# Ced3-han/PepFlowww

Hardware: AMD Instinct MI355X
Metric: residues x denoise-steps / s (higher is better)
Workload: dtype f32 (fp32 storage and accumulation; matrix products as 3 x f16 split MFMA, ~22-bit operands); 1 GPU; cfg4/GPU: B=64 x 128-residue synthetic pockets (112 ctx + 16 gen) per GPU; per_gpu_batch=64, residues=128, global_batch=64, parallelism=batch-shard x1, hipgraph=True, precision=fp32

## Files before the change

### pepflowww_amd/csrc/common.h

```cpp
#pragma once
#include <hip/hip_runtime.h>

static inline int pf_cu_count() {
    static int cache[64] = {0};
    int dev = 0, c = 256;
    if (hipGetDevice(&dev) != hipSuccess) return 256;
    if (dev >= 0 && dev < 64 && cache[dev] > 0) return cache[dev];
    if (hipDeviceGetAttribute(&c, hipDeviceAttributeMultiprocessorCount, dev) != hipSuccess || c <= 0) c = 256;
    if (dev >= 0 && dev < 64) cache[dev] = c;
    return c;
}
#include <stdint.h>

#define PF_WAVE 64

typedef float f32x4 __attribute__((ext_vector_type(4)));

__device__ __forceinline__ f32x4 mfma16(float a, float b, f32x4 c) {
    return __builtin_amdgcn_mfma_f32_16x16x4f32(a, b, c, 0, 0, 0);
}

__device__ __forceinline__ void lds_barrier() {
    asm volatile("s_waitcnt lgkmcnt(0)" ::: "memory");
    __builtin_amdgcn_s_barrier();
    asm volatile("" ::: "memory");
}

template <int CTRL, int BANK = 0xF>
__device__ __forceinline__ float dpp_mov(float old, float v) {
    return __int_as_float(__builtin_amdgcn_update_dpp(__float_as_int(old), __float_as_int(v), CTRL, 0xF, BANK, false));
}
__device__ __forceinline__ float lane_xor1(float v) { return dpp_mov<0xB1>(v, v); }
__device__ __forceinline__ float lane_xor2(float v) { return dpp_mov<0x4E>(v, v); }
__device__ __forceinline__ float lane_xor4(float v) {
    float t = dpp_mov<0x104, 0x5>(v, v);
    return dpp_mov<0x114, 0xA>(t, v);
}
__device__ __forceinline__ float lane_xor8(float v) { return dpp_mov<0x128>(v, v); }
template <int OFF> __device__ __forceinline__ float lane_xor(float v) {
    if constexpr (OFF == 1) return lane_xor1(v);
    else if constexpr (OFF == 2) return lane_xor2(v);
    else if constexpr (OFF == 4) return lane_xor4(v);
    else return lane_xor8(v);
}
__device__ __forceinline__ float sum_xor16(float v) {
    auto r = __builtin_amdgcn_permlane16_swap(__float_as_uint(v), __float_as_uint(v), false, false);
    return __uint_as_float(r[0]) + __uint_as_float(r[1]);
}
__device__ __forceinline__ float sum_xor32(float v) {
    auto r = __builtin_amdgcn_permlane32_swap(__float_as_uint(v), __float_as_uint(v), false, false);
    return __uint_as_float(r[0]) + __uint_as_float(r[1]);
}
__device__ __forceinline__ float max_xor16(float v) {
    auto r = __builtin_amdgcn_permlane16_swap(__float_as_uint(v), __float_as_uint(v), false, false);
    return fmaxf(__uint_as_float(r[0]), __uint_as_float(r[1]));
}
__device__ __forceinline__ float max_xor32(float v) {
    auto r = __builtin_amdgcn_permlane32_swap(__float_as_uint(v), __float_as_uint(v), false, false);
    return fmaxf(__uint_as_float(r[0]), __uint_as_float(r[1]));
}
__device__ __forceinline__ bool pf_rows_all_masked(const int* __restrict__ key_end, int L, int m0, int n, int M) {
    if (!key_end) return false;
    const int mend = m0 + n < M ? m0 + n : M;
    int m = m0;
    while (m < mend) {
        const int b = m / L, i = m - b * L;
        if (i < key_end[b]) return false;
        m = (b + 1) * L;
    }
    return true;
}
__device__ __forceinline__ float row16_sum(float v) {
    v += lane_xor8(v); v += lane_xor4(v); v += lane_xor2(v); v += lane_xor1(v);
    return v;
}
__device__ __forceinline__ float row16_max(float v) {
    v = fmaxf(v, lane_xor8(v)); v = fmaxf(v, lane_xor4(v)); v = fmaxf(v, lane_xor2(v)); v = fmaxf(v, lane_xor1(v));
    return v;
}
__device__ __forceinline__ float wave_sum(float v) { return sum_xor32(sum_xor16(row16_sum(v))); }
__device__ __forceinline__ float wave_max(float v) { return max_xor32(max_xor16(row16_max(v))); }

__device__ __forceinline__ float keep_if(bool ok, float v) { return __uint_as_float(__float_as_uint(v) & (ok ? 0xffffffffu : 0u)); }
__device__ __forceinline__ float4 keep_if(bool ok, const float4& v) {
    const unsigned m = ok ? 0xffffffffu : 0u;
    return make_float4(__uint_as_float(__float_as_uint(v.x) & m), __uint_as_float(__float_as_uint(v.y) & m),
                       __uint_as_float(__float_as_uint(v.z) & m), __uint_as_float(__float_as_uint(v.w) & m));
}

template <int MT, int NT>
__device__ __forceinline__ void mfma_slice(const float4 (&a)[MT], const float4 (&b)[NT], f32x4 (&acc)[MT][NT]) {
#pragma unroll
    for (int mt = 0; mt < MT; ++mt)
#pragma unroll
        for (int nt = 0; nt < NT; ++nt) {
            acc[mt][nt] = mfma16(a[mt].x, b[nt].x, acc[mt][nt]);
            acc[mt][nt] = mfma16(a[mt].y, b[nt].y, acc[mt][nt]);
            acc[mt][nt] = mfma16(a[mt].z, b[nt].z, acc[mt][nt]);
            acc[mt][nt] = mfma16(a[mt].w, b[nt].w, acc[mt][nt]);
        }
}

template <int NT, int PF_DEPTH = 4>
struct BStream {
    const float* wrow[NT];
    bool wok[NT];
    float4 ring[PF_DEPTH][NT];
    int nslices;

    __device__ __forceinline__ void init(const float* __restrict__ W, int ldw, int n0, int n_valid, int K) {
        const int lane = threadIdx.x & 63;
        const int r = lane & 15, g = lane >> 4;
        nslices = K >> 4;
#pragma unroll
        for (int nt = 0; nt < NT; ++nt) {
            const int n = n0 + 16 * nt + r;
            wok[nt] = n < n_valid;
            wrow[nt] = W + (size_t)(wok[nt] ? n : 0) * ldw + 4 * g;
        }
    }
    __device__ __forceinline__ void load(int slot_static, int slice, float4 (&dst)[NT]) {
        (void)slot_static;
#pragma unroll
        for (int nt = 0; nt < NT; ++nt)
            dst[nt] = *reinterpret_cast<const float4*>(wrow[nt] + 16 * slice);
    }
    __device__ __forceinline__ void prefetch() {
#pragma unroll
        for (int d = 0; d < PF_DEPTH; ++d)
            if (d < nslices) load(d, d, ring[d]);
    }
};

template <int MT, int NT, int PF_DEPTH>
__device__ __forceinline__ void gemm_ldsA_stream(const float* __restrict__ A_lds, int lda, BStream<NT, PF_DEPTH>& bs,
                                                 f32x4 (&acc)[MT][NT], int slice0, int count) {
    const int lane = threadIdx.x & 63;
    const float* arow = A_lds + (lane & 15) * lda + 4 * (lane >> 4);
    const int ns = bs.nslices;
    for (int base = 0; base < count; base += PF_DEPTH) {
#pragma unroll
        for (int u = 0; u < PF_DEPTH; ++u) {
            if (base + u < count) {
                const int sl = slice0 + base + u;
                float4 a[MT];
#pragma unroll
                for (int mt = 0; mt < MT; ++mt)
                    a[mt] = *reinterpret_cast<const float4*>(arow + mt * 16 * lda + 16 * (base + u));
                mfma_slice<MT, NT>(a, bs.ring[u], acc);
                if (sl + PF_DEPTH < ns) bs.load(u, sl + PF_DEPTH, bs.ring[u]);
            }
        }
    }
}

template <int MT, int NT>
__device__ __forceinline__ void gemm_ldsA_glbB(const float* __restrict__ A_lds, int lda,
                                               const float* __restrict__ W, int ldw, int n0, int n_valid,
                                               int K, f32x4 (&acc)[MT][NT]) {
    BStream<NT> bs;
    bs.init(W, ldw, n0, n_valid, K);
    bs.prefetch();
    gemm_ldsA_stream<MT, NT, 4>(A_lds, lda, bs, acc, 0, bs.nslices);
}

typedef _Float16 half8 __attribute__((ext_vector_type(8)));
typedef _Float16 half4 __attribute__((ext_vector_type(4)));
__device__ __forceinline__ float exp_softmax(float x) { return __builtin_amdgcn_exp2f(x * 1.4426950408889634f); }
constexpr float PF_LO_SCALE = 2048.f, PF_LO_INV = 1.f / 2048.f;

__device__ __forceinline__ f32x4 mfma_h(half8 a, half8 b, f32x4 c) {
    return __builtin_amdgcn_mfma_f32_16x16x32_f16(a, b, c, 0, 0, 0);
}
constexpr float PF_F16_MAX = 65504.f;
#ifndef PF_SPLIT_SATURATE
#define PF_SPLIT_SATURATE 1
#endif
__device__ __forceinline__ void split4(const float (&v)[4], half4& hi, half4& lo) {
#pragma unroll
    for (int e = 0; e < 4; ++e) {
#if PF_SPLIT_SATURATE
        const float vc = fminf(fmaxf(v[e], -PF_F16_MAX), PF_F16_MAX) + v[e] * 0.f;
#else
        const float vc = v[e];
#endif
        const _Float16 h = (_Float16)vc;
        hi[e] = h;
        lo[e] = (_Float16)__builtin_fmaf((float)h, -PF_LO_SCALE, vc * PF_LO_SCALE);
    }
}
__device__ __forceinline__ float join(f32x4 m, f32x4 c, int e) { return m[e] + c[e] * PF_LO_INV; }

template <int WT, int D, bool SP = false>
struct WSplit {
    const _Float16* wh[WT];
    const _Float16* wl[WT];
    half8 rh[D][WT], rl[D][WT];
    int nsteps;
    __device__ __forceinline__ void init(const void* planes, int Npad, int K, int n0) {
        const int lane = threadIdx.x & 63;
        const _Float16* hi = reinterpret_cast<const _Float16*>(planes);
        const _Float16* lo = hi + (size_t)Npad * K;
        nsteps = K >> 5;
#pragma unroll
        for (int wt = 0; wt < WT; ++wt) {
            const size_t off = ((size_t)((n0 >> 4) + wt) * nsteps * 64 + lane) * 8;
            wh[wt] = hi + off;
            wl[wt] = lo + off;
        }
    }
    __device__ __forceinline__ void load(int step, half8 (&dh)[WT], half8 (&dl)[WT]) {
#pragma unroll
        for (int wt = 0; wt < WT; ++wt) {
            dh[wt] = *reinterpret_cast<const half8*>(wh[wt] + (size_t)step * 512);
            if constexpr (!SP) dl[wt] = *reinterpret_cast<const half8*>(wl[wt] + (size_t)step * 512);
        }
    }
    __device__ __forceinline__ void prefetch() {
#pragma unroll
        for (int d = 0; d < D; ++d)
            if (d < nsteps) load(d, rh[d], rl[d]);
    }
};

template <int WT, int D, bool SP>
__device__ __forceinline__ void gemm_split16(WSplit<WT, D, SP>& ws, const _Float16* Xh, const _Float16* Xl, int ldx,
                                             f32x4 (&am)[WT], f32x4 (&ac)[WT], int step0, int count) {
    const int lane = threadIdx.x & 63;
    const int off = (lane & 15) * ldx + 8 * (lane >> 4);
    for (int base = 0; base < count; base += D) {
#pragma unroll
        for (int u = 0; u < D; ++u) {
            if (base + u < count) {
                const int st = step0 + base + u;
                const half8 xh = *reinterpret_cast<const half8*>(Xh + off + 32 * (base + u));
                half8 xl;
                if constexpr (!SP) xl = *reinterpret_cast<const half8*>(Xl + off + 32 * (base + u));
#pragma unroll
                for (int wt = 0; wt < WT; ++wt) {
                    am[wt] = mfma_h(ws.rh[u][wt], xh, am[wt]);
                    if constexpr (!SP) {
                        ac[wt] = mfma_h(ws.rh[u][wt], xl, ac[wt]);
                        ac[wt] = mfma_h(ws.rl[u][wt], xh, ac[wt]);
                    }
                }
                if (st + D < ws.nsteps) ws.load(st + D, ws.rh[u], ws.rl[u]);
            }
        }
    }
}
template <int WT, int D, bool SP, int RT>
__device__ __forceinline__ void gemm_split16r(WSplit<WT, D, SP>& ws, const _Float16* Xh, const _Float16* Xl, int ldx,
                                              f32x4 (&am)[RT][WT], f32x4 (&ac)[RT][WT], int step0, int count) {
    const int lane = threadIdx.x & 63;
    const int off = (lane & 15) * ldx + 8 * (lane >> 4);
    for (int base = 0; base < count; base += D) {
#pragma unroll
        for (int u = 0; u < D; ++u) {
            if (base + u < count) {
                const int st = step0 + base + u;
#pragma unroll
                for (int rt = 0; rt < RT; ++rt) {
                    const half8 xh = *reinterpret_cast<const half8*>(Xh + rt * 16 * ldx + off + 32 * (base + u));
                    half8 xl;
                    if constexpr (!SP) xl = *reinterpret_cast<const half8*>(Xl + rt * 16 * ldx + off + 32 * (base + u));
#pragma unroll
                    for (int wt = 0; wt < WT; ++wt) {
                        am[rt][wt] = mfma_h(ws.rh[u][wt], xh, am[rt][wt]);
                        if constexpr (!SP) {
                            ac[rt][wt] = mfma_h(ws.rh[u][wt], xl, ac[rt][wt]);
                            ac[rt][wt] = mfma_h(ws.rl[u][wt], xh, ac[rt][wt]);
                        }
                    }
                }
                if (st + D < ws.nsteps) ws.load(st + D, ws.rh[u], ws.rl[u]);
            }
        }
    }
}
template <int WT> __device__ __forceinline__ void acc_zero1(f32x4 (&a)[WT], f32x4 (&b)[WT]) {
#pragma unroll
    for (int wt = 0; wt < WT; ++wt) { a[wt] = (f32x4){0.f, 0.f, 0.f, 0.f}; b[wt] = (f32x4){0.f, 0.f, 0.f, 0.f}; }
}

template <int WT>
struct WPre {
    half8 h[WT], l[WT];
    __device__ __forceinline__ void load(const void* planes, int N, int Kw, int n0) {
        const int lane = threadIdx.x & 63;
        const int wsteps = Kw >> 5;
        const _Float16* wh = reinterpret_cast<const _Float16*>(planes) + ((size_t)(n0 >> 4) * wsteps * 64 + lane) * 8;
        const _Float16* wl = wh + (size_t)N * Kw;
        const size_t tstride = (size_t)wsteps * 512;
#pragma unroll
        for (int wt = 0; wt < WT; ++wt) {
            h[wt] = *reinterpret_cast<const half8*>(wh + wt * tstride);
            l[wt] = *reinterpret_cast<const half8*>(wl + wt * tstride);
        }
    }
};

template <int WT, int PT, bool SP = false>
__device__ __forceinline__ void gemm_split_lowreg(const void* planes, int N, int Kw, int n0, int K,
                                                  const _Float16* Xh, const _Float16* Xl, int ldx,
                                                  f32x4 (&am)[WT][PT], f32x4 (&ac)[WT][PT]) {
    static_assert(PT % 2 == 0, "row tiles are fed in pairs");
    const int lane = threadIdx.x & 63, r = lane & 15, g = lane >> 4;
    const int wsteps = Kw >> 5, nst = K >> 5;
    const _Float16* wh = reinterpret_cast<const _Float16*>(planes) + ((size_t)(n0 >> 4) * wsteps * 64 + lane) * 8;
    const _Float16* wl = wh + (size_t)N * Kw;
    const size_t tstride = (size_t)wsteps * 512;
    const _Float16* xh = Xh + r * ldx + 8 * g;
    const _Float16* xl = Xl + r * ldx + 8 * g;
    for (int st = 0; st < nst; ++st) {
        half8 bh[WT], bl[WT];
#pragma unroll
        for (int wt = 0; wt < WT; ++wt) {
            bh[wt] = *reinterpret_cast<const half8*>(wh + wt * tstride + (size_t)st * 512);
            if constexpr (!SP) bl[wt] = *reinterpret_cast<const half8*>(wl + wt * tstride + (size_t)st * 512);
        }
#pragma unroll
        for (int p0 = 0; p0 < PT; p0 += 2) {
            half8 ah[2], al[2];
#pragma unroll
            for (int q = 0; q < 2; ++q) {
                ah[q] = *reinterpret_cast<const half8*>(xh + (p0 + q) * 16 * ldx + 32 * st);
                if constexpr (!SP) al[q] = *reinterpret_cast<const half8*>(xl + (p0 + q) * 16 * ldx + 32 * st);
            }
#pragma unroll
            for (int wt = 0; wt < WT; ++wt)
#pragma unroll
                for (int q = 0; q < 2; ++q) am[wt][p0 + q] = mfma_h(bh[wt], ah[q], am[wt][p0 + q]);
            if constexpr (!SP) {
#pragma unroll
                for (int wt = 0; wt < WT; ++wt)
#pragma unroll
                    for (int q = 0; q < 2; ++q) ac[wt][p0 + q] = mfma_h(bh[wt], al[q], ac[wt][p0 + q]);
#pragma unroll
                for (int wt = 0; wt < WT; ++wt)
#pragma unroll
                    for (int q = 0; q < 2; ++q) ac[wt][p0 + q] = mfma_h(bl[wt], ah[q], ac[wt][p0 + q]);
            }
        }
    }
}

template <int WT, int PT, bool SWZ = false, bool SP = false, bool SWAP = false>
__device__ __forceinline__ void gemm_split(const void* planes, int N, int Kw, int n0, int K,
                                           const _Float16* Xh, const _Float16* Xl, int ldx,
                                           f32x4 (&am)[WT][PT], f32x4 (&ac)[WT][PT], const WPre<WT>* pre = nullptr) {
    const int lane = threadIdx.x & 63, r = lane & 15, g = lane >> 4;
    const int wsteps = Kw >> 5;
    const _Float16* wh = reinterpret_cast<const _Float16*>(planes) + ((size_t)(n0 >> 4) * wsteps * 64 + lane) * 8;
    const _Float16* wl = wh + (size_t)N * Kw;
    const size_t tstride = (size_t)wsteps * 512;
    const int gs = SWZ ? (g ^ ((r >> 2) & 1)) : g;
    const _Float16* xh = Xh + r * ldx + 8 * gs;
    const _Float16* xl = Xl + r * ldx + 8 * gs;
    half8 bh[WT], bl[WT], nh[WT], nl[WT];
#pragma unroll
    for (int wt = 0; wt < WT; ++wt) {
        if (pre) { bh[wt] = pre->h[wt]; bl[wt] = pre->l[wt]; }
        else {
            bh[wt] = *reinterpret_cast<const half8*>(wh + wt * tstride);
            if constexpr (!SP) bl[wt] = *reinterpret_cast<const half8*>(wl + wt * tstride);
        }
    }
    const int nst = K >> 5;
    for (int st = 0; st < nst; ++st) {
        if (st + 1 < nst) {
#pragma unroll
            for (int wt = 0; wt < WT; ++wt) {
                nh[wt] = *reinterpret_cast<const half8*>(wh + wt * tstride + (size_t)(st + 1) * 512);
                if constexpr (!SP) nl[wt] = *reinterpret_cast<const half8*>(wl + wt * tstride + (size_t)(st + 1) * 512);
            }
        }
        half8 ah[PT], al[PT];
#pragma unroll
        for (int pt = 0; pt < PT; ++pt) {
            ah[pt] = *reinterpret_cast<const half8*>(xh + pt * 16 * ldx + 32 * st);
            if constexpr (!SP) al[pt] = *reinterpret_cast<const half8*>(xl + pt * 16 * ldx + 32 * st);
        }
#pragma unroll
        for (int wt = 0; wt < WT; ++wt)
#pragma unroll
            for (int pt = 0; pt < PT; ++pt) am[wt][pt] = SWAP ? mfma_h(ah[pt], bh[wt], am[wt][pt]) : mfma_h(bh[wt], ah[pt], am[wt][pt]);
        if constexpr (!SP) {
#pragma unroll
            for (int wt = 0; wt < WT; ++wt)
#pragma unroll
                for (int pt = 0; pt < PT; ++pt) ac[wt][pt] = SWAP ? mfma_h(al[pt], bh[wt], ac[wt][pt]) : mfma_h(bh[wt], al[pt], ac[wt][pt]);
#pragma unroll
            for (int wt = 0; wt < WT; ++wt)
#pragma unroll
                for (int pt = 0; pt < PT; ++pt) ac[wt][pt] = SWAP ? mfma_h(ah[pt], bl[wt], ac[wt][pt]) : mfma_h(bl[wt], ah[pt], ac[wt][pt]);
        }
#pragma unroll
        for (int wt = 0; wt < WT; ++wt) { bh[wt] = nh[wt]; if constexpr (!SP) bl[wt] = nl[wt]; }
    }
}

__device__ __forceinline__ int swz_col(int n0, int r, int g) {
    return n0 + 8 * ((g >> 1) ^ ((r >> 2) & 1)) + 4 * (g & 1);
}

template <int MT, int NT>
__device__ __forceinline__ void acc_zero(f32x4 (&acc)[MT][NT]) {
#pragma unroll
    for (int mt = 0; mt < MT; ++mt)
#pragma unroll
        for (int nt = 0; nt < NT; ++nt) acc[mt][nt] = (f32x4){0.f, 0.f, 0.f, 0.f};
}

__device__ __forceinline__ int xcd_remap(int bid, int nblk) {
    const int q = nblk >> 3, rem = nblk & 7, x = bid & 7, k = bid >> 3;
    return (x < rem ? x * (q + 1) : rem * (q + 1) + (x - rem) * q) + k;
}

#define PF_CHECK_LAUNCH() do { hipError_t e_ = hipGetLastError(); if (e_ != hipSuccess) return (int)e_; } while (0)

struct PfOncePerDevice {
    bool done[32] = {};
    bool first() {
        int d = 0;
        (void)hipGetDevice(&d);
        d &= 31;
        if (done[d]) return false;
        done[d] = true;
        return true;
    }
};
```

### pepflowww_amd/csrc/node_track.hip

```cpp
#include "common.h"
#include "rigid_dev.h"
#include "../../include/pepflow_hip.h"

#ifdef PF_PROFILE
__device__ long long g_prof[64];
#ifndef PF_PROF_LAST
#define PF_PROF_LAST 1
#endif
#define PROF(i) do { if (LAST == (PF_PROF_LAST != 0) && blockIdx.x == 0 && threadIdx.x == 0) g_prof[i] = clock64(); } while (0)
extern "C" int pf_debug_prof(long long* out, int n) {
    return (int)hipMemcpyFromSymbol(out, HIP_SYMBOL(g_prof), sizeof(long long) * n, 0, hipMemcpyDeviceToHost);
}
#else
#define PROF(i)
#endif

namespace {

constexpr int TR = 16;
constexpr int LDX = 132;
constexpr int LDP = 136;
constexpr int NTHR = 512;
#ifndef PF_NT_MINW
#define PF_NT_MINW 2
#endif

struct Planes { _Float16* h; _Float16* l; };

struct LnParams { float g[8], b[8]; };
__device__ __forceinline__ void ln_load(LnParams& p, const float* __restrict__ g, const float* __restrict__ b) {
    const int sub = threadIdx.x & 15;
    const float4 g0 = *reinterpret_cast<const float4*>(g + 8 * sub), g1 = *reinterpret_cast<const float4*>(g + 8 * sub + 4);
    const float4 b0 = *reinterpret_cast<const float4*>(b + 8 * sub), b1 = *reinterpret_cast<const float4*>(b + 8 * sub + 4);
    p.g[0] = g0.x; p.g[1] = g0.y; p.g[2] = g0.z; p.g[3] = g0.w; p.g[4] = g1.x; p.g[5] = g1.y; p.g[6] = g1.z; p.g[7] = g1.w;
    p.b[0] = b0.x; p.b[1] = b0.y; p.b[2] = b0.z; p.b[3] = b0.w; p.b[4] = b1.x; p.b[5] = b1.y; p.b[6] = b1.z; p.b[7] = b1.w;
}
template <int ROWS = 16>
__device__ __forceinline__ void ln_tile(float* T, const LnParams& p, float mk, Planes out, int m0, int M, float* gout) {
    const int tid = threadIdx.x;
    if (tid < 16 * ROWS) {
        const int row = tid >> 4, sub = tid & 15, m = m0 + row;
        float v[8];
        {
            const float4 a = *reinterpret_cast<const float4*>(T + row * LDX + 8 * sub);
            const float4 b = *reinterpret_cast<const float4*>(T + row * LDX + 8 * sub + 4);
            v[0] = a.x; v[1] = a.y; v[2] = a.z; v[3] = a.w; v[4] = b.x; v[5] = b.y; v[6] = b.z; v[7] = b.w;
        }
        float s = ((v[0] + v[1]) + (v[2] + v[3])) + ((v[4] + v[5]) + (v[6] + v[7]));
        s = row16_sum(s);
        const float mean = s / 128.f;
        float q = 0.f;
#pragma unroll
        for (int c = 0; c < 8; ++c) { const float d = v[c] - mean; q += d * d; }
        q = row16_sum(q);
        const float rstd = rsqrtf(q / 128.f + 1e-5f);
        float y[8];
#pragma unroll
        for (int c = 0; c < 8; ++c) y[c] = ((v[c] - mean) * rstd * p.g[c] + p.b[c]) * mk;
        *reinterpret_cast<float4*>(T + row * LDX + 8 * sub) = make_float4(y[0], y[1], y[2], y[3]);
        *reinterpret_cast<float4*>(T + row * LDX + 8 * sub + 4) = make_float4(y[4], y[5], y[6], y[7]);
        half4 h0, l0, h1, l1;
        const float y0[4] = {y[0], y[1], y[2], y[3]}, y1[4] = {y[4], y[5], y[6], y[7]};
        split4(y0, h0, l0);
        split4(y1, h1, l1);
        *reinterpret_cast<half4*>(out.h + row * LDP + 8 * sub) = h0;
        *reinterpret_cast<half4*>(out.h + row * LDP + 8 * sub + 4) = h1;
        *reinterpret_cast<half4*>(out.l + row * LDP + 8 * sub) = l0;
        *reinterpret_cast<half4*>(out.l + row * LDP + 8 * sub + 4) = l1;
        if (gout && m < M) {
            *reinterpret_cast<float4*>(gout + (size_t)m * 128 + 8 * sub) = make_float4(y[0], y[1], y[2], y[3]);
            *reinterpret_cast<float4*>(gout + (size_t)m * 128 + 8 * sub + 4) = make_float4(y[4], y[5], y[6], y[7]);
        }
    }
}

__device__ __forceinline__ float4 sel4(bool ok, const float4& v) {
    const float f = ok ? 1.f : 0.f;
    return make_float4(v.x * f, v.y * f, v.z * f, v.w * f);
}

__device__ __forceinline__ void put_planes(Planes p, int r, int n, const float (&v)[4]) {
    half4 hi, lo;
    split4(v, hi, lo);
    *reinterpret_cast<half4*>(p.h + r * LDP + n) = hi;
    *reinterpret_cast<half4*>(p.l + r * LDP + n) = lo;
}

template <bool SP, bool DUMP = false, bool PM = false>
__global__ __launch_bounds__(NTHR, PF_NT_MINW) void node_head_kernel(pf_node_head_args a) {
    extern __shared__ __attribute__((aligned(16))) unsigned char smem_raw[];
    constexpr int CK = 256, LDC = CK + 8;
    _Float16* Ch = reinterpret_cast<_Float16*>(smem_raw);
    float* X = reinterpret_cast<float*>(smem_raw + 2 * 2 * TR * LDC * sizeof(_Float16));
    Planes Xa = {reinterpret_cast<_Float16*>(X + TR * LDX), reinterpret_cast<_Float16*>(X + TR * LDX) + TR * LDP};
    const int tid = threadIdx.x, wave = tid >> 6, lane = tid & 63;
    const int r = lane & 15, g = lane >> 4;
    const int m0 = blockIdx.x * TR, M = a.rows;
    if (pf_rows_all_masked(a.key_end, a.key_L, m0, TR, M)) return;
    const int n = wave * 16 + 4 * g;

    constexpr int C0 = PM ? 4 : 0;
    WSplit<1, 8, SP> ws;
    ws.init(a.w_out_f16, 128, PF_IPA_FEATS - C0 * 256, wave * 16);
    ws.prefetch();
    LnParams lnp;
    ln_load(lnp, a.ln_g, a.ln_b);
    const float4 bias_out = *reinterpret_cast<const float4*>(a.b_out + n);
    float4 bias_in[3];
#pragma unroll
    for (int wt = 0; wt < 3; ++wt) bias_in[wt] = *reinterpret_cast<const float4*>(a.b_in + wave * 48 + wt * 16 + 4 * g);
    const int mr = m0 + r;
    const int mrc = mr < M ? mr : M - 1;
    const float rmask_ld = a.mask[mrc];
    const float4 rres_ld = *reinterpret_cast<const float4*>(a.s_in + (size_t)mrc * 128 + n);
    const int srow = tid >> 5, sc4 = tid & 31;
    const bool sok = m0 + srow < M;
    const float* src = a.feats + (size_t)(sok ? m0 + srow : 0) * PF_IPA_FEATS + 4 * sc4;
    constexpr int NCH = PF_IPA_FEATS / CK;
    float4 st[NCH][2];
#pragma unroll
    for (int c = 0; c < NCH; ++c)
#pragma unroll
        for (int hlf = 0; hlf < 2; ++hlf)
            st[c][hlf] = *reinterpret_cast<const float4*>(src + c * CK + hlf * 128);
    auto commit = [&](int c) {
        _Float16* bh = Ch + (c & 1) * 2 * TR * LDC;
        _Float16* bl = bh + TR * LDC;
#pragma unroll
        for (int hlf = 0; hlf < 2; ++hlf) {
            const float4 sv = sel4(sok, st[c][hlf]);
            const float v[4] = {sv.x, sv.y, sv.z, sv.w};
            half4 hi, lo;
            split4(v, hi, lo);
            *reinterpret_cast<half4*>(bh + srow * LDC + hlf * 128 + 4 * sc4) = hi;
            *reinterpret_cast<half4*>(bl + srow * LDC + hlf * 128 + 4 * sc4) = lo;
        }
    };
    if constexpr (PM) {
        auto add4 = [](const float4& p, const float4& q) { return make_float4(p.x + q.x, p.y + q.y, p.z + q.z, p.w + q.w); };
        float4 ev = sel4(sok, st[0][0]), od = sel4(sok, st[0][1]);
#pragma unroll
        for (int c = 1; c < 4; ++c) { ev = add4(ev, sel4(sok, st[c][0])); od = add4(od, sel4(sok, st[c][1])); }
        *reinterpret_cast<float4*>(X + srow * LDX + 4 * sc4) = add4(ev, od);
    }
    commit(C0);
    __syncthreads();
    f32x4 am[1], ac[1];
    acc_zero1<1>(am, ac);
#pragma unroll
    for (int c = C0; c < NCH; ++c) {
        const _Float16* bh = Ch + (c & 1) * 2 * TR * LDC;
        gemm_split16(ws, bh, bh + TR * LDC, LDC, am, ac, (c - C0) * 8, 8);
        if (c + 1 < NCH) commit(c + 1);
        __syncthreads();
    }
    WSplit<3, 4, SP> wq;
    wq.init(a.w_in_f16, 384, 128, wave * 48);
    wq.prefetch();
    {
        const float rmask = rmask_ld * (mr < M ? 1.f : 0.f);
        const float4 rres = sel4(mr < M, rres_ld);
        float4 hs = make_float4(0.f, 0.f, 0.f, 0.f);
        if constexpr (PM) hs = *reinterpret_cast<const float4*>(X + r * LDX + n);
        auto lin = [&](int e, float h) { const float j = join(am[0], ac[0], e); if constexpr (PM) return j + h; else return j; };
        float4 y;
        y.x = (lin(0, hs.x) + bias_out.x) * rmask + rres.x;
        y.y = (lin(1, hs.y) + bias_out.y) * rmask + rres.y;
        y.z = (lin(2, hs.z) + bias_out.z) * rmask + rres.z;
        y.w = (lin(3, hs.w) + bias_out.w) * rmask + rres.w;
        *reinterpret_cast<float4*>(X + r * LDX + n) = y;
        if constexpr (DUMP) { if (mr < M) *reinterpret_cast<float4*>(a.dump_a0 + (size_t)mr * 128 + n) = y; }
    }
    __syncthreads();
    ln_tile(X, lnp, 1.f, Xa, m0, M, a.s_ipa);
    __syncthreads();
    f32x4 qm[3], qc[3];
    acc_zero1<3>(qm, qc);
    gemm_split16(wq, Xa.h, Xa.l, LDP, qm, qc, 0, 4);
    if (mr < M) {
#pragma unroll
        for (int wt = 0; wt < 3; ++wt) {
            float4 y;
            y.x = join(qm[wt], qc[wt], 0) + bias_in[wt].x; y.y = join(qm[wt], qc[wt], 1) + bias_in[wt].y;
            y.z = join(qm[wt], qc[wt], 2) + bias_in[wt].z; y.w = join(qm[wt], qc[wt], 3) + bias_in[wt].w;
            *reinterpret_cast<float4*>(a.qkv + (size_t)mr * 384 + wave * 48 + wt * 16 + 4 * g) = y;
        }
    }
}

constexpr int TR2 = 32;
template <bool SP, bool PM = false>
__global__ __launch_bounds__(NTHR, PF_NT_MINW) void node_head32_kernel(pf_node_head_args a) {
    extern __shared__ __attribute__((aligned(16))) unsigned char smem_raw[];
    constexpr int CK = 256, LDC = CK + 8;
    _Float16* Ch = reinterpret_cast<_Float16*>(smem_raw);
    float* X = reinterpret_cast<float*>(smem_raw + 2 * 2 * TR2 * LDC * sizeof(_Float16));
    Planes Xa = {reinterpret_cast<_Float16*>(X + TR2 * LDX), reinterpret_cast<_Float16*>(X + TR2 * LDX) + TR2 * LDP};
    const int tid = threadIdx.x, wave = tid >> 6, lane = tid & 63;
    const int r = lane & 15, g = lane >> 4;
    int m0 = blockIdx.x * TR2, M = a.rows;
    if (a.key_end) {
        const int tps = (a.key_L + TR2 - 1) / TR2, b = blockIdx.x / tps, i0 = (blockIdx.x - b * tps) * TR2;
        if (i0 >= a.key_end[b]) return;
        m0 = b * a.key_L + i0;
        M = (b + 1) * a.key_L;
    }
    const int n = wave * 16 + 4 * g;

    constexpr int C0 = PM ? 4 : 0;
    WSplit<1, 8, SP> ws;
    ws.init(a.w_out_f16, 128, PF_IPA_FEATS - C0 * 256, wave * 16);
    ws.prefetch();
    LnParams lnp;
    ln_load(lnp, a.ln_g, a.ln_b);
    const float4 bias_out = *reinterpret_cast<const float4*>(a.b_out + n);
    float4 bias_in[3];
#pragma unroll
    for (int wt = 0; wt < 3; ++wt) bias_in[wt] = *reinterpret_cast<const float4*>(a.b_in + wave * 48 + wt * 16 + 4 * g);
    float rmask_ld[2];
    float4 rres_ld[2];
#pragma unroll
    for (int rt = 0; rt < 2; ++rt) {
        const int mr = m0 + rt * 16 + r;
        const int mrc = mr < M ? mr : M - 1;
        rmask_ld[rt] = a.mask[mrc];
        rres_ld[rt] = *reinterpret_cast<const float4*>(a.s_in + (size_t)mrc * 128 + n);
    }
    constexpr int NCH = PF_IPA_FEATS / CK;
    float4 st[2][4];
    auto fetch = [&](int c, float4 (&d)[4]) {
#pragma unroll
        for (int u = 0; u < 4; ++u) {
            const int idx = tid + u * NTHR, row = idx >> 6, c4 = idx & 63;
            const int m = m0 + row < M ? m0 + row : M - 1;
            d[u] = *reinterpret_cast<const float4*>(a.feats + (size_t)m * PF_IPA_FEATS + c * CK + 4 * c4);
        }
    };
    auto commit = [&](int c, const float4 (&d)[4]) {
        _Float16* bh = Ch + (c & 1) * 2 * TR2 * LDC;
        _Float16* bl = bh + TR2 * LDC;
#pragma unroll
        for (int u = 0; u < 4; ++u) {
            const int idx = tid + u * NTHR, row = idx >> 6, c4 = idx & 63;
            const float4 sv = sel4(m0 + row < M, d[u]);
            const float v[4] = {sv.x, sv.y, sv.z, sv.w};
            half4 hi, lo;
            split4(v, hi, lo);
            *reinterpret_cast<half4*>(bh + row * LDC + 4 * c4) = hi;
            *reinterpret_cast<half4*>(bl + row * LDC + 4 * c4) = lo;
        }
    };
    fetch(0, st[0]);
    fetch(1, st[1]);
    if constexpr (PM) {
        auto add4 = [](const float4& p, const float4& q) { return make_float4(p.x + q.x, p.y + q.y, p.z + q.z, p.w + q.w); };
        float4 hsum[4];
#pragma unroll
        for (int c = 0; c < 4; ++c) {
#pragma unroll
            for (int u = 0; u < 4; ++u) {
                const int idx = tid + u * NTHR, row = idx >> 6;
                const float4 v = sel4(m0 + row < M, st[c & 1][u]);
                hsum[u] = c == 0 ? v : add4(hsum[u], v);
            }
            fetch(c + 2, st[c & 1]);
        }
#pragma unroll
        for (int u = 0; u < 4; ++u) {
            const int idx = tid + u * NTHR, row = idx >> 6, c4 = idx & 63;
            float4 o;
            o.x = __shfl_xor(hsum[u].x, 32); o.y = __shfl_xor(hsum[u].y, 32); o.z = __shfl_xor(hsum[u].z, 32); o.w = __shfl_xor(hsum[u].w, 32);
            if (c4 < 32) *reinterpret_cast<float4*>(X + row * LDX + 4 * c4) = add4(hsum[u], o);
        }
    }
    commit(C0, st[C0 & 1]);
    __syncthreads();
    f32x4 am[2][1], ac[2][1];
#pragma unroll
    for (int rt = 0; rt < 2; ++rt) acc_zero1<1>(am[rt], ac[rt]);
#pragma unroll
    for (int c = C0; c < NCH; ++c) {
        if (!PM && c + 2 < NCH) fetch(c + 2, st[c & 1]);
        const _Float16* bh = Ch + (c & 1) * 2 * TR2 * LDC;
        gemm_split16r<1, 8, SP, 2>(ws, bh, bh + TR2 * LDC, LDC, am, ac, (c - C0) * 8, 8);
        if (c + 1 < NCH) commit(c + 1, st[(c + 1) & 1]);
        __syncthreads();
    }
    WSplit<3, 4, SP> wq;
    wq.init(a.w_in_f16, 384, 128, wave * 48);
    wq.prefetch();
#pragma unroll
    for (int rt = 0; rt < 2; ++rt) {
        const int mr = m0 + rt * 16 + r;
        const float rmask = rmask_ld[rt] * (mr < M ? 1.f : 0.f);
        const float4 rres = sel4(mr < M, rres_ld[rt]);
        float4 hs = make_float4(0.f, 0.f, 0.f, 0.f);
        if constexpr (PM) hs = *reinterpret_cast<const float4*>(X + (rt * 16 + r) * LDX + n);
        auto lin = [&](int e, float h) { const float j = join(am[rt][0], ac[rt][0], e); if constexpr (PM) return j + h; else return j; };
        float4 y;
        y.x = (lin(0, hs.x) + bias_out.x) * rmask + rres.x;
        y.y = (lin(1, hs.y) + bias_out.y) * rmask + rres.y;
        y.z = (lin(2, hs.z) + bias_out.z) * rmask + rres.z;
        y.w = (lin(3, hs.w) + bias_out.w) * rmask + rres.w;
        *reinterpret_cast<float4*>(X + (rt * 16 + r) * LDX + n) = y;
    }
    __syncthreads();
    ln_tile<TR2>(X, lnp, 1.f, Xa, m0, M, a.s_ipa);
    __syncthreads();
    f32x4 qm[2][3], qc[2][3];
#pragma unroll
    for (int rt = 0; rt < 2; ++rt) acc_zero1<3>(qm[rt], qc[rt]);
    gemm_split16r<3, 4, SP, 2>(wq, Xa.h, Xa.l, LDP, qm, qc, 0, 4);
#pragma unroll
    for (int rt = 0; rt < 2; ++rt) {
        const int mr = m0 + rt * 16 + r;
        if (mr < M) {
#pragma unroll
            for (int wt = 0; wt < 3; ++wt) {
                float4 y;
                y.x = join(qm[rt][wt], qc[rt][wt], 0) + bias_in[wt].x; y.y = join(qm[rt][wt], qc[rt][wt], 1) + bias_in[wt].y;
                y.z = join(qm[rt][wt], qc[rt][wt], 2) + bias_in[wt].z; y.w = join(qm[rt][wt], qc[rt][wt], 3) + bias_in[wt].w;
                *reinterpret_cast<float4*>(a.qkv + (size_t)mr * 384 + wave * 48 + wt * 16 + 4 * g) = y;
            }
        }
    }
}

template <bool LAST, bool SP, int RT, bool DUMP = false>
__global__ __launch_bounds__(NTHR, PF_NT_MINW) void node_tfmr_kernel(pf_node_tfmr_args a, int LP, int LDS_S) {
    constexpr int TR = 16 * RT;
    extern __shared__ __attribute__((aligned(16))) float smem[];
    float* T0 = smem;
    float* T1 = T0 + TR * LDX;
    float* U = T1 + TR * LDX;
    _Float16* pl = reinterpret_cast<_Float16*>(U + TR * 8);
    Planes Xa = {pl, pl + TR * LDP}, Xb = {pl + 2 * TR * LDP, pl + 3 * TR * LDP};
    float* S = reinterpret_cast<float*>(pl + 4 * TR * LDP);
    const int tid = threadIdx.x, wave = tid >> 6, lane = tid & 63;
    const int r = lane & 15, g = lane >> 4;
    const int L = a.L;
    const int tiles = (L + TR - 1) / TR;
    const int lid = a.key_end ? (int)blockIdx.x : xcd_remap(blockIdx.x, gridDim.x);
    const int b = lid / tiles;
    const int i0 = (lid - b * tiles) * TR;
    const size_t rowb = (size_t)b * L;
    if (a.key_end && i0 >= __builtin_amdgcn_readfirstlane(a.key_end[b])) return;
    if constexpr (LAST) {
        if (a.row_on) {
            int any = 0;
#pragma unroll
            for (int rt = 0; rt < RT; ++rt) any |= a.row_on[((int)rowb + min(i0 + 16 * rt, L - 16)) >> 4];
            if (!__builtin_amdgcn_readfirstlane(any)) return;
        }
    }
    const int m0 = (int)rowb + i0;
    const int M = (int)rowb + L;
    const int n = wave * 16 + 4 * g;
    int mr[RT];
#pragma unroll
    for (int rt = 0; rt < RT; ++rt) mr[rt] = m0 + 16 * rt + r;
    auto dump4 = [&](float* p, int rt, float x, float y, float z, float w) {
        if constexpr (DUMP) { if (mr[rt] < M) *reinterpret_cast<float4*>(p + (size_t)mr[rt] * 128 + n) = make_float4(x, y, z, w); }
    };

    PROF(0);
    const int h = wave & 3;
    float4 q0[RT], q1[RT];
#pragma unroll
    for (int rt = 0; rt < RT; ++rt) {
        const int i = i0 + 16 * rt + r;
        const float* qrow = a.qkv + (rowb + (i < L ? i : 0)) * 384 + h * 32 + 4 * g;
        q0[rt] = *reinterpret_cast<const float4*>(qrow);
        q1[rt] = *reinterpret_cast<const float4*>(qrow + 16);
    }
    const float4 z4 = make_float4(0.f, 0.f, 0.f, 0.f);
    const int par = wave >> 2;
    auto kload = [&](int j0, float4 (&k0)[2], float4 (&k1)[2], float (&km)[2]) {
#pragma unroll
        for (int t = 0; t < 2; ++t) {
            const int j = j0 + 32 * t + r;
            const int jc = j < L ? j : L - 1;
            const float* krow = a.qkv + (rowb + jc) * 384 + 128 + h * 32 + 4 * g;
            k0[t] = *reinterpret_cast<const float4*>(krow);
            k1[t] = *reinterpret_cast<const float4*>(krow + 16);
            km[t] = a.mask[rowb + jc];
        }
    };
    float4 kfA0[2], kfA1[2], kfB0[2], kfB1[2];
    float kfAm[2], kfBm[2];
    kload(16 * par, kfA0, kfA1, kfAm);
    kload(16 * par + 64, kfB0, kfB1, kfBm);
    asm volatile("" ::: "memory");
    const int ct = wave >> 2;
    const float* vcol = a.qkv + rowb * 384 + 256 + h * 32 + ct * 16 + r;
    auto vload = [&](int k0, float (&vb)[4][4]) {
#pragma unroll
        for (int s4 = 0; s4 < 4; ++s4)
#pragma unroll
            for (int t = 0; t < 4; ++t) {
                int j = k0 + 16 * s4 + 4 * g + t;
                j = j < L ? j : L - 1;
                vb[s4][t] = vcol[(size_t)j * 384];
            }
    };
    float vbA[4][4], vbB[4][4];
    vload(0, vbA);
    vload(64, vbB);
    asm volatile("" ::: "memory");
    WSplit<1, 4, SP> ws;
    ws.init(a.w_o_f16, 128, 128, wave * 16);
    ws.prefetch();
    LnParams ln1, ln2, ln3;
    ln_load(ln1, a.n1_g, a.n1_b);
    ln_load(ln2, a.n2_g, a.n2_b);
    if (LAST) ln_load(ln3, a.nt_g, a.nt_b);
    const float4 bias_o = *reinterpret_cast<const float4*>(a.b_o + n), bias_1 = *reinterpret_cast<const float4*>(a.b_1 + n),
                 bias_2 = *reinterpret_cast<const float4*>(a.b_2 + n);
    float4 bias_post = z4, bias_t1 = z4, bias_t2 = z4, bias_t3 = z4, bias_bb = z4, bias_init = z4;
    float4 bias_in[3] = {z4, z4, z4}, bias_pre[4] = {z4, z4, z4, z4};
    float4 rres_ld[RT], rsipa_ld[RT];
#pragma unroll
    for (int rt = 0; rt < RT; ++rt) {
        const int mrc = mr[rt] < M ? mr[rt] : M - 1;
        rres_ld[rt] = *reinterpret_cast<const float4*>(a.resid + (size_t)mrc * 128 + n);
        rsipa_ld[rt] = LAST ? *reinterpret_cast<const float4*>(a.s_ipa + (size_t)mrc * 128 + n) : z4;
    }
    float lnmask_ld = 1.f;
    const int lnrow = m0 + ((tid & (16 * TR - 1)) >> 4);
    auto load_tail_consts = [&]() {
        bias_post = *reinterpret_cast<const float4*>(a.b_post + n);
        bias_t1 = *reinterpret_cast<const float4*>(a.b_t1 + n);
        bias_t2 = *reinterpret_cast<const float4*>(a.b_t2 + n);
        bias_t3 = *reinterpret_cast<const float4*>(a.b_t3 + n);
        bias_bb = *reinterpret_cast<const float4*>(a.b_bb + 4 * (g & 1));
        if (a.has_et) {
            bias_init = *reinterpret_cast<const float4*>(a.b_init + (wave & 3) * 16 + 4 * g);
#pragma unroll
            for (int wt = 0; wt < 4; ++wt) bias_pre[wt] = *reinterpret_cast<const float4*>(a.b_pre + wave * 64 + wt * 16 + 4 * g);
        }
        lnmask_ld = a.mask[lnrow < M ? lnrow : M - 1];
    };
    if (LAST) {
        if (RT == 1) load_tail_consts();
    } else {
#pragma unroll
        for (int wt = 0; wt < 3; ++wt) bias_in[wt] = *reinterpret_cast<const float4*>(a.b_in_next + wave * 48 + wt * 16 + 4 * g);
    }

    PROF(1);
    {
        const float scale = 0.17677669529663687f;
        auto score_block = [&](int j0, const float4 (&k0)[2], const float4 (&k1)[2], const float (&km)[2]) {
#pragma unroll
            for (int t = 0; t < 2; ++t) {
                const int j = j0 + 32 * t + r;
                if (j0 + 32 * t < LP) {
                    const bool keep = j < L && km[t] > 0.5f;
#pragma unroll
                    for (int rt = 0; rt < RT; ++rt) {
                        f32x4 acc = {0.f, 0.f, 0.f, 0.f};
                        acc = mfma16(q0[rt].x, k0[t].x, acc); acc = mfma16(q0[rt].y, k0[t].y, acc); acc = mfma16(q0[rt].z, k0[t].z, acc); acc = mfma16(q0[rt].w, k0[t].w, acc);
                        acc = mfma16(q1[rt].x, k1[t].x, acc); acc = mfma16(q1[rt].y, k1[t].y, acc); acc = mfma16(q1[rt].z, k1[t].z, acc); acc = mfma16(q1[rt].w, k1[t].w, acc);
#pragma unroll
                        for (int e = 0; e < 4; ++e) S[((16 * rt + 4 * g + e) * 4 + h) * LDS_S + j] = keep ? acc[e] * scale : -3.0e38f;
                    }
                }
            }
        };
        score_block(16 * par, kfA0, kfA1, kfAm);
        if (16 * par + 64 < LP) score_block(16 * par + 64, kfB0, kfB1, kfBm);
        for (int j0 = 16 * par + 128; j0 < LP; j0 += 64) {
            float4 kn0[2], kn1[2];
            float knm[2];
            kload(j0, kn0, kn1, knm);
            score_block(j0, kn0, kn1, knm);
        }
    }
    __syncthreads();
    PROF(2);
#pragma unroll
    for (int ps = 0; ps < RT; ++ps) {
        const int sub = lane & 7;
        float* sp = S + ((ps * 8 + wave) * 8 + (lane >> 3)) * LDS_S;
        if (LP <= 256) {
            float4 v[8];
#pragma unroll
            for (int u = 0; u < 8; ++u) {
                const int j = 4 * sub + 32 * u;
                v[u] = j < LP ? *reinterpret_cast<const float4*>(sp + j) : make_float4(-3.0e38f, -3.0e38f, -3.0e38f, -3.0e38f);
            }
            float m = -3.0e38f;
#pragma unroll
            for (int u = 0; u < 8; ++u) m = fmaxf(m, fmaxf(fmaxf(v[u].x, v[u].y), fmaxf(v[u].z, v[u].w)));
            m = fmaxf(m, lane_xor1(m)); m = fmaxf(m, lane_xor2(m)); m = fmaxf(m, lane_xor4(m));
            float sum = 0.f;
#pragma unroll
            for (int u = 0; u < 8; ++u) {
                v[u].x = (v[u].x > -1.0e38f) ? exp_softmax(v[u].x - m) : 0.f; v[u].y = (v[u].y > -1.0e38f) ? exp_softmax(v[u].y - m) : 0.f;
                v[u].z = (v[u].z > -1.0e38f) ? exp_softmax(v[u].z - m) : 0.f; v[u].w = (v[u].w > -1.0e38f) ? exp_softmax(v[u].w - m) : 0.f;
                sum += (v[u].x + v[u].y) + (v[u].z + v[u].w);
            }
            sum += lane_xor1(sum); sum += lane_xor2(sum); sum += lane_xor4(sum);
            const float inv = 1.f / sum;
#pragma unroll
            for (int u = 0; u < 8; ++u) {
                const int j = 4 * sub + 32 * u;
                if (j < LP) *reinterpret_cast<float4*>(sp + j) = make_float4(v[u].x * inv, v[u].y * inv, v[u].z * inv, v[u].w * inv);
            }
        } else {
            float m = -3.0e38f;
            for (int j = sub; j < LP; j += 8) m = fmaxf(m, sp[j]);
            m = fmaxf(m, lane_xor1(m)); m = fmaxf(m, lane_xor2(m)); m = fmaxf(m, lane_xor4(m));
            float sum = 0.f;
            for (int j = sub; j < LP; j += 8) { const float e = (sp[j] > -1.0e38f) ? exp_softmax(sp[j] - m) : 0.f; sp[j] = e; sum += e; }
            sum += lane_xor1(sum); sum += lane_xor2(sum); sum += lane_xor4(sum);
            const float inv = 1.f / sum;
            for (int j = sub; j < LP; j += 8) sp[j] *= inv;
        }
    }
    __syncthreads();
    PROF(3);
    {
        f32x4 acc[RT];
#pragma unroll
        for (int rt = 0; rt < RT; ++rt) acc[rt] = (f32x4){0.f, 0.f, 0.f, 0.f};
        const float* prow = S + (r * 4 + h) * LDS_S + 4 * g;
        auto pv_block = [&](int k0, const float (&vb)[4][4]) {
#pragma unroll
            for (int s4 = 0; s4 < 4; ++s4) {
                if (k0 + 16 * s4 < LP) {
#pragma unroll
                    for (int rt = 0; rt < RT; ++rt) {
                        const float4 pa = *reinterpret_cast<const float4*>(prow + rt * 64 * LDS_S + k0 + 16 * s4);
                        acc[rt] = mfma16(pa.x, vb[s4][0], acc[rt]); acc[rt] = mfma16(pa.y, vb[s4][1], acc[rt]);
                        acc[rt] = mfma16(pa.z, vb[s4][2], acc[rt]); acc[rt] = mfma16(pa.w, vb[s4][3], acc[rt]);
                    }
                }
            }
        };
        pv_block(0, vbA);
        if (64 < LP) pv_block(64, vbB);
        for (int k0 = 128; k0 < LP; k0 += 64) {
            float vn[4][4];
            vload(k0, vn);
            pv_block(k0, vn);
        }
        const int col = h * 32 + ct * 16 + r;
#pragma unroll
        for (int rt = 0; rt < RT; ++rt)
#pragma unroll
            for (int e = 0; e < 4; ++e) {
                const _Float16 hi = (_Float16)acc[rt][e];
                Xa.h[(16 * rt + 4 * g + e) * LDP + col] = hi;
                Xa.l[(16 * rt + 4 * g + e) * LDP + col] = (_Float16)((acc[rt][e] - (float)hi) * PF_LO_SCALE);
                if constexpr (DUMP) { if (m0 + 16 * rt + 4 * g + e < M) a.dump[0][(size_t)(m0 + 16 * rt + 4 * g + e) * 128 + col] = acc[rt][e]; }
            }
    }
    if (LAST && RT == 2) load_tail_consts();
    __syncthreads();
    PROF(4);

    f32x4 am[RT][1], ac[RT][1];
    auto zero = [&]() {
#pragma unroll
        for (int rt = 0; rt < RT; ++rt) acc_zero1<1>(am[rt], ac[rt]);
    };
    auto joined = [&](int rt, const float4& bias, float (&v)[4]) {
        v[0] = join(am[rt][0], ac[rt][0], 0) + bias.x; v[1] = join(am[rt][0], ac[rt][0], 1) + bias.y;
        v[2] = join(am[rt][0], ac[rt][0], 2) + bias.z; v[3] = join(am[rt][0], ac[rt][0], 3) + bias.w;
    };
    auto relu4 = [](float (&v)[4]) {
#pragma unroll
        for (int e = 0; e < 4; ++e) v[e] = fmaxf(v[e], 0.f);
    };
    zero();
    gemm_split16r<1, 4, SP, RT>(ws, Xa.h, Xa.l, LDP, am, ac, 0, 4);
    ws.init(a.w_1_f16, 128, 128, wave * 16);
    ws.prefetch();
#pragma unroll
    for (int rt = 0; rt < RT; ++rt) {
        const float4 rres = sel4(mr[rt] < M, rres_ld[rt]);
        float v[4];
        joined(rt, bias_o, v);
        *reinterpret_cast<float4*>(T1 + (16 * rt + r) * LDX + n) = make_float4(v[0] + rres.x, v[1] + rres.y, v[2] + rres.z, v[3] + rres.w);
        dump4(a.dump[1], rt, v[0] + rres.x, v[1] + rres.y, v[2] + rres.z, v[3] + rres.w);
    }
    __syncthreads();
    ln_tile<TR>(T1, ln1, 1.f, Xb, m0, M, DUMP ? a.dump[2] : nullptr);
    __syncthreads();
    PROF(5);
    zero();
    gemm_split16r<1, 4, SP, RT>(ws, Xb.h, Xb.l, LDP, am, ac, 0, 4);
    ws.init(a.w_2_f16, 128, 128, wave * 16);
    ws.prefetch();
#pragma unroll
    for (int rt = 0; rt < RT; ++rt) {
        float v[4];
        joined(rt, bias_1, v);
        relu4(v);
        put_planes(Xa, 16 * rt + r, n, v);
        dump4(a.dump[3], rt, v[0], v[1], v[2], v[3]);
    }
    __syncthreads();
    PROF(6);
    zero();
    gemm_split16r<1, 4, SP, RT>(ws, Xa.h, Xa.l, LDP, am, ac, 0, 4);
    auto lin2_to_t0 = [&]() {
#pragma unroll
        for (int rt = 0; rt < RT; ++rt) {
            const float4 u = *reinterpret_cast<const float4*>(T1 + (16 * rt + r) * LDX + n);
            float v[4];
            joined(rt, bias_2, v);
            *reinterpret_cast<float4*>(T0 + (16 * rt + r) * LDX + n) = make_float4(v[0] + u.x, v[1] + u.y, v[2] + u.z, v[3] + u.w);
            dump4(a.dump[4], rt, v[0] + u.x, v[1] + u.y, v[2] + u.z, v[3] + u.w);
        }
    };
    if constexpr (!LAST) {
        WSplit<3, 4, SP> wq;
        wq.init(a.w_in_next_f16, 384, 128, wave * 48);
        wq.prefetch();
        lin2_to_t0();
        __syncthreads();
        ln_tile<TR>(T0, ln2, 1.f, Xb, m0, M, a.v_out);
        __syncthreads();
        PROF(7);
        f32x4 qm[RT][3], qc[RT][3];
#pragma unroll
        for (int rt = 0; rt < RT; ++rt) acc_zero1<3>(qm[rt], qc[rt]);
        gemm_split16r<3, 4, SP, RT>(wq, Xb.h, Xb.l, LDP, qm, qc, 0, 4);
#pragma unroll
        for (int rt = 0; rt < RT; ++rt) {
            if (mr[rt] < M) {
#pragma unroll
                for (int wt = 0; wt < 3; ++wt) {
                    float4 y;
                    y.x = join(qm[rt][wt], qc[rt][wt], 0) + bias_in[wt].x; y.y = join(qm[rt][wt], qc[rt][wt], 1) + bias_in[wt].y;
                    y.z = join(qm[rt][wt], qc[rt][wt], 2) + bias_in[wt].z; y.w = join(qm[rt][wt], qc[rt][wt], 3) + bias_in[wt].w;
                    *reinterpret_cast<float4*>(a.qkv_out + (size_t)mr[rt] * 384 + wave * 48 + wt * 16 + 4 * g) = y;
                }
            }
        }
        PROF(8);
    } else {
        ws.init(a.w_post_f16, 128, 128, wave * 16);
        ws.prefetch();
        lin2_to_t0();
        float4 fq = make_float4(1.f, 0.f, 0.f, 0.f);
        float fR[9], fx[3], fmask = 0.f;
        if (tid < TR && m0 + tid < M) {
            const int m = m0 + tid;
            fq = *reinterpret_cast<const float4*>(a.quat_in + (size_t)m * 4);
#pragma unroll
            for (int k = 0; k < 9; ++k) fR[k] = a.rot_in[(size_t)m * 9 + k];
#pragma unroll
            for (int k = 0; k < 3; ++k) fx[k] = a.trans_in[(size_t)m * 3 + k];
            fmask = a.mask[m];
        }
        __syncthreads();
        ln_tile<TR>(T0, ln2, 1.f, Xb, m0, M, DUMP ? a.dump[5] : nullptr);
        __syncthreads();
        PROF(7);
        zero();
        gemm_split16r<1, 4, SP, RT>(ws, Xb.h, Xb.l, LDP, am, ac, 0, 4);
        ws.init(a.w_t1_f16, 128, 128, wave * 16);
        ws.prefetch();
#pragma unroll
        for (int rt = 0; rt < RT; ++rt) {
            const float4 rsipa = sel4(mr[rt] < M, rsipa_ld[rt]);
            float v[4];
            joined(rt, bias_post, v);
            v[0] += rsipa.x; v[1] += rsipa.y; v[2] += rsipa.z; v[3] += rsipa.w;
            *reinterpret_cast<float4*>(T1 + (16 * rt + r) * LDX + n) = make_float4(v[0], v[1], v[2], v[3]);
            put_planes(Xa, 16 * rt + r, n, v);
            dump4(a.dump[6], rt, v[0], v[1], v[2], v[3]);
        }
        __syncthreads();
        PROF(8);
        zero();
        gemm_split16r<1, 4, SP, RT>(ws, Xa.h, Xa.l, LDP, am, ac, 0, 4);
        ws.init(a.w_t2_f16, 128, 128, wave * 16);
        ws.prefetch();
#pragma unroll
        for (int rt = 0; rt < RT; ++rt) {
            float v[4];
            joined(rt, bias_t1, v);
            relu4(v);
            put_planes(Xb, 16 * rt + r, n, v);
            dump4(a.dump[7], rt, v[0], v[1], v[2], v[3]);
        }
        __syncthreads();
        zero();
        gemm_split16r<1, 4, SP, RT>(ws, Xb.h, Xb.l, LDP, am, ac, 0, 4);
        ws.init(a.w_t3_f16, 128, 128, wave * 16);
        ws.prefetch();
#pragma unroll
        for (int rt = 0; rt < RT; ++rt) {
            float v[4];
            joined(rt, bias_t2, v);
            relu4(v);
            put_planes(Xa, 16 * rt + r, n, v);
            dump4(a.dump[8], rt, v[0], v[1], v[2], v[3]);
        }
        __syncthreads();
        zero();
        gemm_split16r<1, 4, SP, RT>(ws, Xa.h, Xa.l, LDP, am, ac, 0, 4);
        const bool do_bb = wave == 0, do_init = a.has_et && wave >= 4;
        if (do_bb) { ws.init(a.w_bb_f16, 16, 128, 0); ws.prefetch(); }
        else if (do_init) { ws.init(a.w_init_f16, 64, 128, (wave - 4) * 16); ws.prefetch(); }
        WSplit<4, 2, SP> wp;
        if (a.has_et) { wp.init(a.w_pre_f16, PF_ET_PRE, 64, wave * 64); wp.prefetch(); }
#pragma unroll
        for (int rt = 0; rt < RT; ++rt) {
            const float4 s0 = *reinterpret_cast<const float4*>(T1 + (16 * rt + r) * LDX + n);
            float v[4];
            joined(rt, bias_t3, v);
            *reinterpret_cast<float4*>(T0 + (16 * rt + r) * LDX + n) = make_float4(v[0] + s0.x, v[1] + s0.y, v[2] + s0.z, v[3] + s0.w);
            dump4(a.dump[9], rt, v[0] + s0.x, v[1] + s0.y, v[2] + s0.z, v[3] + s0.w);
        }
        __syncthreads();
        ln_tile<TR>(T0, ln3, lnmask_ld * (lnrow < M ? 1.f : 0.f), Xb, m0, M, a.s_out);
        __syncthreads();
        PROF(9);
        if (do_bb || do_init) {
            zero();
            gemm_split16r<1, 4, SP, RT>(ws, Xb.h, Xb.l, LDP, am, ac, 0, 4);
#pragma unroll
            for (int rt = 0; rt < RT; ++rt) {
                float v[4];
                if (do_bb) {
                    joined(rt, bias_bb, v);
                    if (g < 2) *reinterpret_cast<float4*>(U + (16 * rt + r) * 8 + 4 * g) = make_float4(v[0], v[1], v[2], v[3]);
                    if constexpr (DUMP) { if (g < 2 && mr[rt] < M) *reinterpret_cast<float4*>(a.dump[10] + (size_t)mr[rt] * 8 + 4 * g) = make_float4(v[0], v[1], v[2], v[3]); }
                } else {
                    joined(rt, bias_init, v);
                    put_planes(Xa, 16 * rt + r, (wave - 4) * 16 + 4 * g, v);
                }
            }
        }
        __syncthreads();
        if (tid < TR && m0 + tid < M) {
            const int m = m0 + tid;
            float Ro[9], xo[3];
            float4 qo;
            rigid_update_dev(fq, fR, fx, U + tid * 8, fmask, qo, Ro, xo);
            *reinterpret_cast<float4*>(a.quat_out + (size_t)m * 4) = qo;
#pragma unroll
            for (int k = 0; k < 3; ++k) a.trans_out[(size_t)m * 3 + k] = xo[k];
#pragma unroll
            for (int k = 0; k < 9; ++k) a.rot_out[(size_t)m * 9 + k] = Ro[k];
        }
        PROF(10);
        if (a.has_et) {
            f32x4 pm[RT][4], pc[RT][4];
#pragma unroll
            for (int rt = 0; rt < RT; ++rt) acc_zero1<4>(pm[rt], pc[rt]);
            PROF(12);
            gemm_split16r<4, 2, SP, RT>(wp, Xa.h, Xa.l, LDP, pm, pc, 0, 2);
            PROF(13);
#pragma unroll
            for (int rt = 0; rt < RT; ++rt) {
                if (mr[rt] < M) {
#pragma unroll
                    for (int wt = 0; wt < 4; ++wt) {
                        float4 y;
                        y.x = join(pm[rt][wt], pc[rt][wt], 0) + bias_pre[wt].x; y.y = join(pm[rt][wt], pc[rt][wt], 1) + bias_pre[wt].y;
                        y.z = join(pm[rt][wt], pc[rt][wt], 2) + bias_pre[wt].z; y.w = join(pm[rt][wt], pc[rt][wt], 3) + bias_pre[wt].w;
                        *reinterpret_cast<float4*>(a.pre + (size_t)mr[rt] * PF_ET_PRE + wave * 64 + wt * 16 + 4 * g) = y;
                    }
                }
            }
        } else if (a.logits_out) {
            __syncthreads();
            Planes Xc = {reinterpret_cast<_Float16*>(T0), reinterpret_cast<_Float16*>(T0) + TR * LDP};
#pragma unroll
            for (int net = 0; net < 2; ++net) {
                const int nout = net ? 5 : 20, ntile = net ? 1 : 2;
                ws.init(a.h_w[net][0], 128, 128, wave * 16);
                ws.prefetch();
                const float4 hb0 = *reinterpret_cast<const float4*>(a.h_b[net][0] + n), hb1 = *reinterpret_cast<const float4*>(a.h_b[net][1] + n);
                zero();
                gemm_split16r<1, 4, SP, RT>(ws, Xb.h, Xb.l, LDP, am, ac, 0, 4);
                ws.init(a.h_w[net][1], 128, 128, wave * 16);
                ws.prefetch();
#pragma unroll
                for (int rt = 0; rt < RT; ++rt) {
                    float v[4];
                    joined(rt, hb0, v);
                    relu4(v);
                    put_planes(Xa, 16 * rt + r, n, v);
                }
                __syncthreads();
                zero();
                gemm_split16r<1, 4, SP, RT>(ws, Xa.h, Xa.l, LDP, am, ac, 0, 4);
                if (wave < ntile) { ws.init(a.h_w[net][2], 16 * ntile, 128, wave * 16); ws.prefetch(); }
#pragma unroll
                for (int rt = 0; rt < RT; ++rt) {
                    float v[4];
                    joined(rt, hb1, v);
                    relu4(v);
                    put_planes(Xc, 16 * rt + r, n, v);
                }
                __syncthreads();
                if (wave < ntile) {
                    const float4 hb2 = *reinterpret_cast<const float4*>(a.h_b[net][2] + n);
                    zero();
                    gemm_split16r<1, 4, SP, RT>(ws, Xc.h, Xc.l, LDP, am, ac, 0, 4);
#pragma unroll
                    for (int rt = 0; rt < RT; ++rt) {
                        if (mr[rt] < M) {
                            float* op = (net ? a.ang_out : a.logits_out) + (size_t)mr[rt] * nout;
                            float v[4];
                            joined(rt, hb2, v);
#pragma unroll
                            for (int e = 0; e < 4; ++e)
                                if (n + e < nout) op[n + e] = v[e];
                        }
                    }
                }
                __syncthreads();
            }
        }
        PROF(11);
    }
}

constexpr int LDF = 640 + 8;
template <bool SP>
__global__ __launch_bounds__(NTHR) void input_mixer_kernel(pf_input_mixer_args a) {
    extern __shared__ __attribute__((aligned(16))) unsigned char smem_raw[];
    Planes Xf = {reinterpret_cast<_Float16*>(smem_raw), reinterpret_cast<_Float16*>(smem_raw) + TR * LDF};
    Planes Xa = {Xf.l + TR * LDF, Xf.l + TR * LDF + TR * LDP};
    const int tid = threadIdx.x, wave = tid >> 6, lane = tid & 63;
    const int r = lane & 15, g = lane >> 4;
    const int m0 = blockIdx.x * TR, M = a.B * a.L;
    const int n = wave * 16 + 4 * g;
    WSplit<1, 8, SP> w0;
    w0.init(a.w0_f16, 128, 640, wave * 16);
    w0.prefetch();
    const float4 b0 = *reinterpret_cast<const float4*>(a.b0 + n);
    const float4 b2 = *reinterpret_cast<const float4*>(a.b2 + n);
    const int mr = m0 + r, mrc = mr < M ? mr : M - 1;
    const float rmask = a.mask[mrc] * (mr < M ? 1.f : 0.f);
    __shared__ float TC[2][128];
    const int b_first = m0 / a.L, b_last = min(m0 + TR - 1, M - 1) / a.L;
    const bool tc_shared = b_last - b_first < 2;
    if (tc_shared && tid < 128 * (b_last - b_first + 1)) {
        const int bi = tid >> 7, k = tid & 127;
        const float tt = a.t[b_first + bi] * 2056.f;
        TC[bi][k] = k < 64 ? sinf(tt * a.time_freq[k]) : cosf(tt * a.time_freq[k - 64]);
    }
    __syncthreads();
    for (int idx = tid; idx < TR * 160; idx += NTHR) {
        const int row = idx / 160, c4 = idx - row * 160;
        const int m = min(m0 + row, M - 1);
        const int b = m / a.L;
        float v[4];
        if (c4 < 32) {
            const float4 t = *reinterpret_cast<const float4*>(a.node_embed + (size_t)m * 128 + 4 * c4);
            v[0] = t.x; v[1] = t.y; v[2] = t.z; v[3] = t.w;
        } else if (c4 < 64) {
            long long sq = a.seqs[m];
            sq = sq < 0 ? 0 : (sq > 21 ? 21 : sq);
            const float4 t = *reinterpret_cast<const float4*>(a.seq_table + sq * 128 + 4 * (c4 - 32));
            v[0] = t.x; v[1] = t.y; v[2] = t.z; v[3] = t.w;
        } else {
            const float tt = a.t[b] * 2056.f;
#pragma unroll
            for (int e = 0; e < 4; ++e) {
                const int c = 4 * c4 + e;
                float x;
                if (c < 384 && tc_shared) x = TC[b - b_first][c - 256];
                else if (c < 320) x = sinf(tt * a.time_freq[c - 256]);
                else if (c < 384) x = cosf(tt * a.time_freq[c - 320]);
                else if (c < 629) {
                    const int q = c - 384, d = q / 49, k = q - d * 49;
                    const float ang = a.angles[(size_t)m * 5 + d];
                    if (k == 0) x = ang;
                    else if (k < 25) x = sinf(ang * a.ang_freq[k - 1]);
                    else x = cosf(ang * a.ang_freq[k - 25]);
                } else x = 0.f;
                v[e] = x;
            }
        }
        half4 hi, lo;
        split4(v, hi, lo);
        *reinterpret_cast<half4*>(Xf.h + row * LDF + 4 * c4) = hi;
        *reinterpret_cast<half4*>(Xf.l + row * LDF + 4 * c4) = lo;
    }
    if (tid < TR && m0 + tid < M) {
        float R[9], q[4];
#pragma unroll
        for (int k = 0; k < 9; ++k) R[k] = a.rot[(size_t)(m0 + tid) * 9 + k];
        rot_to_quat_dev(R, q);
        *reinterpret_cast<float4*>(a.quat + (size_t)(m0 + tid) * 4) = make_float4(q[0], q[1], q[2], q[3]);
    }
    __syncthreads();
    f32x4 am[1], ac[1];
    acc_zero1<1>(am, ac);
    gemm_split16(w0, Xf.h, Xf.l, LDF, am, ac, 0, 20);
    WSplit<1, 4, SP> w2;
    w2.init(a.w2_f16, 128, 128, wave * 16);
    w2.prefetch();
    {
        const float v[4] = {fmaxf(join(am[0], ac[0], 0) + b0.x, 0.f), fmaxf(join(am[0], ac[0], 1) + b0.y, 0.f),
                            fmaxf(join(am[0], ac[0], 2) + b0.z, 0.f), fmaxf(join(am[0], ac[0], 3) + b0.w, 0.f)};
        put_planes(Xa, r, n, v);
    }
    __syncthreads();
    acc_zero1<1>(am, ac);
    gemm_split16(w2, Xa.h, Xa.l, LDP, am, ac, 0, 4);
    if (mr < M) {
        float4 y;
        y.x = (join(am[0], ac[0], 0) + b2.x) * rmask; y.y = (join(am[0], ac[0], 1) + b2.y) * rmask;
        y.z = (join(am[0], ac[0], 2) + b2.z) * rmask; y.w = (join(am[0], ac[0], 3) + b2.w) * rmask;
        *reinterpret_cast<float4*>(a.s_out + (size_t)mr * 128 + n) = y;
    }
}

}

extern "C" int pf_input_mixer_fwd(const pf_input_mixer_args* a, pf_stream_t stream) {
    if (!a || !a->node_embed || !a->seq_table || !a->seqs || !a->t || !a->time_freq || !a->ang_freq || !a->angles || !a->w0_f16 ||
        !a->b0 || !a->w2_f16 || !a->b2 || !a->mask || !a->rot || !a->quat || !a->s_out || a->B <= 0 || a->L <= 0)
        return PF_E_BADARG;
    const int rows = a->B * a->L;
    const size_t lds = (size_t)2 * TR * LDF * sizeof(_Float16) + (size_t)2 * TR * LDP * sizeof(_Float16);
    if (a->single_pass) hipLaunchKernelGGL(input_mixer_kernel<true>, dim3((unsigned)((rows + TR - 1) / TR)), dim3(NTHR), lds, (hipStream_t)stream, *a);
    else hipLaunchKernelGGL(input_mixer_kernel<false>, dim3((unsigned)((rows + TR - 1) / TR)), dim3(NTHR), lds, (hipStream_t)stream, *a);
    PF_CHECK_LAUNCH();
    return 0;
}

extern "C" int pf_node_head_fwd(const pf_node_head_args* a, pf_stream_t stream) {
    if (!a || !a->feats || !a->s_in || !a->mask || !a->w_out_f16 || !a->b_out || !a->ln_g || !a->ln_b || !a->w_in_f16 ||
        !a->b_in || !a->s_ipa || !a->qkv || a->rows <= 0)
        return PF_E_BADARG;
    const size_t lds = (size_t)2 * 2 * TR * 264 * sizeof(_Float16) + (size_t)TR * LDX * sizeof(float) +
                       (size_t)2 * TR * LDP * sizeof(_Float16);
    if (a->rows >= pf_cu_count() * TR2 && !a->dump_a0) {
        const size_t lds2 = (size_t)2 * 2 * TR2 * 264 * sizeof(_Float16) + (size_t)TR2 * LDX * sizeof(float) + (size_t)2 * TR2 * LDP * sizeof(_Float16);
        static PfOncePerDevice attr_set;
        if (attr_set.first()) {
            (void)hipFuncSetAttribute((const void*)node_head32_kernel<true>, hipFuncAttributeMaxDynamicSharedMemorySize, 160 * 1024);
            (void)hipFuncSetAttribute((const void*)node_head32_kernel<false>, hipFuncAttributeMaxDynamicSharedMemorySize, 160 * 1024);
            (void)hipFuncSetAttribute((const void*)node_head32_kernel<true, true>, hipFuncAttributeMaxDynamicSharedMemorySize, 160 * 1024);
            (void)hipFuncSetAttribute((const void*)node_head32_kernel<false, true>, hipFuncAttributeMaxDynamicSharedMemorySize, 160 * 1024);
        }
        const bool per_sample = a->key_end && a->key_L > 0 && a->rows % a->key_L == 0;
        pf_node_head_args aa = *a;
        if (!per_sample) aa.key_end = nullptr;
        const dim3 grid(per_sample ? (unsigned)((a->rows / a->key_L) * ((a->key_L + TR2 - 1) / TR2)) : (unsigned)((a->rows + TR2 - 1) / TR2));
        a = &aa;
        if (a->o_premul) {
            if (a->single_pass) hipLaunchKernelGGL((node_head32_kernel<true, true>), grid, dim3(NTHR), lds2, (hipStream_t)stream, *a);
            else hipLaunchKernelGGL((node_head32_kernel<false, true>), grid, dim3(NTHR), lds2, (hipStream_t)stream, *a);
        } else if (a->single_pass) hipLaunchKernelGGL(node_head32_kernel<true>, grid, dim3(NTHR), lds2, (hipStream_t)stream, *a);
        else hipLaunchKernelGGL(node_head32_kernel<false>, grid, dim3(NTHR), lds2, (hipStream_t)stream, *a);
        PF_CHECK_LAUNCH();
        return 0;
    }
    if (a->dump_a0) {
        if (a->single_pass || a->o_premul) return PF_E_BADARG;
        hipLaunchKernelGGL((node_head_kernel<false, true>), dim3((unsigned)((a->rows + TR - 1) / TR)), dim3(NTHR), lds, (hipStream_t)stream, *a);
        PF_CHECK_LAUNCH();
        return 0;
    }
    if (a->o_premul) {
        if (a->single_pass) hipLaunchKernelGGL((node_head_kernel<true, false, true>), dim3((unsigned)((a->rows + TR - 1) / TR)), dim3(NTHR), lds, (hipStream_t)stream, *a);
        else hipLaunchKernelGGL((node_head_kernel<false, false, true>), dim3((unsigned)((a->rows + TR - 1) / TR)), dim3(NTHR), lds, (hipStream_t)stream, *a);
    } else if (a->single_pass) hipLaunchKernelGGL(node_head_kernel<true>, dim3((unsigned)((a->rows + TR - 1) / TR)), dim3(NTHR), lds, (hipStream_t)stream, *a);
    else hipLaunchKernelGGL(node_head_kernel<false>, dim3((unsigned)((a->rows + TR - 1) / TR)), dim3(NTHR), lds, (hipStream_t)stream, *a);
    PF_CHECK_LAUNCH();
    return 0;
}

extern "C" int pf_node_tfmr_fwd(const pf_node_tfmr_args* a, pf_stream_t stream) {
    if (!a || !a->qkv || !a->resid || !a->mask || !a->w_o_f16 || !a->b_o || !a->n1_g || !a->n1_b || !a->w_1_f16 || !a->b_1 ||
        !a->w_2_f16 || !a->b_2 || !a->n2_g || !a->n2_b || a->B <= 0 || a->L <= 0)
        return PF_E_BADARG;
    if (!a->last && (!a->w_in_next_f16 || !a->b_in_next || !a->qkv_out || !a->v_out)) return PF_E_BADARG;
    if (a->last && (!a->s_ipa || !a->w_post_f16 || !a->b_post || !a->w_t1_f16 || !a->b_t1 || !a->w_t2_f16 || !a->b_t2 ||
                    !a->w_t3_f16 || !a->b_t3 || !a->nt_g || !a->nt_b || !a->w_bb_f16 || !a->b_bb || !a->s_out || !a->quat_in ||
                    !a->rot_in || !a->trans_in || !a->quat_out || !a->rot_out || !a->trans_out))
        return PF_E_BADARG;
    if (a->last && a->has_et && (!a->w_init_f16 || !a->b_init || !a->w_pre_f16 || !a->b_pre || !a->pre)) return PF_E_BADARG;
    if (a->last && !a->has_et && a->logits_out) {
        if (!a->ang_out) return PF_E_BADARG;
        for (int net = 0; net < 2; ++net)
            for (int l = 0; l < 3; ++l)
                if (!a->h_w[net][l] || !a->h_b[net][l]) return PF_E_BADARG;
    }
    const int LP = (a->L + 15) / 16 * 16;
    const int LDS_S = LP + 4;
    const int tiles16 = (a->L + 15) / 16;
    auto lds_of = [&](int rt) {
        const int tr = 16 * rt;
        return ((size_t)2 * tr * LDX + tr * 8 + (size_t)tr * 4 * LDS_S) * sizeof(float) + (size_t)4 * tr * LDP * sizeof(_Float16);
    };
    const int RTn = ((long)a->B * tiles16 > pf_cu_count() && a->L > 16 && !a->dump[0] && lds_of(2) <= (size_t)160 * 1024) ? 2 : 1;
    const int TRn = 16 * RTn;
    const size_t lds = lds_of(RTn);
    if (lds > 160 * 1024) return PF_E_TOOLARGE;
    const int tiles = (a->L + TRn - 1) / TRn;
    const dim3 grid((unsigned)(a->B * tiles));
    const int variant = (RTn == 2 ? 4 : 0) + (a->last ? 2 : 0) + (a->single_pass ? 1 : 0);
    static PfOncePerDevice attr_set[8];
#define PF_NT_CASE(V, LASTV, SPV, RTV)                                                                                           \
    case V:                                                                                                                      \
        if (attr_set[V].first()) {                                                                                                      \
            (void)hipFuncSetAttribute((const void*)node_tfmr_kernel<LASTV, SPV, RTV>, hipFuncAttributeMaxDynamicSharedMemorySize, \
                                      160 * 1024);                                                                               \
        }                                                                                                                        \
        hipLaunchKernelGGL((node_tfmr_kernel<LASTV, SPV, RTV>), grid, dim3(NTHR), lds, (hipStream_t)stream, *a, LP, LDS_S);      \
        break;
    if (a->dump[0]) {
        for (int k = 0; k < (a->last ? 11 : 5); ++k)
            if (!a->dump[k]) return PF_E_BADARG;
        if (a->single_pass || RTn != 1) return PF_E_BADARG;
        static PfOncePerDevice dattr[2];
        if (a->last) {
            if (dattr[1].first()) { (void)hipFuncSetAttribute((const void*)node_tfmr_kernel<true, false, 1, true>, hipFuncAttributeMaxDynamicSharedMemorySize, 160 * 1024); }
            hipLaunchKernelGGL((node_tfmr_kernel<true, false, 1, true>), grid, dim3(NTHR), lds, (hipStream_t)stream, *a, LP, LDS_S);
        } else {
            if (dattr[0].first()) { (void)hipFuncSetAttribute((const void*)node_tfmr_kernel<false, false, 1, true>, hipFuncAttributeMaxDynamicSharedMemorySize, 160 * 1024); }
            hipLaunchKernelGGL((node_tfmr_kernel<false, false, 1, true>), grid, dim3(NTHR), lds, (hipStream_t)stream, *a, LP, LDS_S);
        }
        PF_CHECK_LAUNCH();
        return 0;
    }
    switch (variant) {
        PF_NT_CASE(0, false, false, 1) PF_NT_CASE(1, false, true, 1) PF_NT_CASE(2, true, false, 1) PF_NT_CASE(3, true, true, 1)
        PF_NT_CASE(4, false, false, 2) PF_NT_CASE(5, false, true, 2) PF_NT_CASE(6, true, false, 2) PF_NT_CASE(7, true, true, 2)
    }
#undef PF_NT_CASE
    PF_CHECK_LAUNCH();
    return 0;
}
```

Measured before the change: 2.932 million res*step/s.

## Swizzle LDS layouts for split-f16 planes and attention scores, parallelize logit heads

Adds XOR swizzling to the f16 hi/lo LDS planes, the chunk buffers and the attention score matrix, and changes their padded strides. The aim is to remove LDS bank conflicts in the MFMA operand loads and the softmax/PV reads. It also moves the chain constant loads to after the score phase to relieve register pressure. The two logit/angle head MLPs now run concurrently on separate wave halves using extra LDS planes, instead of running one after the other. The stride changes raise LDS usage, which could affect the RT=2 selection or occupancy, and the swizzle indexing must stay consistent between every writer and reader.

```diff
diff --git a/pepflowww_amd/csrc/common.h b/pepflowww_amd/csrc/common.h
--- a/pepflowww_amd/csrc/common.h
+++ b/pepflowww_amd/csrc/common.h
@@ -223,11 +223,14 @@
     }
 };
 
-template <int WT, int D, bool SP>
+__device__ __forceinline__ int swz_chunk(int chunk, int row) { return chunk ^ ((row >> 2) & 1); }
+__device__ __forceinline__ int swz_at(int col, int row) { return col ^ (((row >> 2) & 1) << 3); }
+
+template <int WT, int D, bool SP, bool SWZ = false>
 __device__ __forceinline__ void gemm_split16(WSplit<WT, D, SP>& ws, const _Float16* Xh, const _Float16* Xl, int ldx,
                                              f32x4 (&am)[WT], f32x4 (&ac)[WT], int step0, int count) {
     const int lane = threadIdx.x & 63;
-    const int off = (lane & 15) * ldx + 8 * (lane >> 4);
+    const int off = (lane & 15) * ldx + 8 * (SWZ ? swz_chunk(lane >> 4, lane & 15) : (lane >> 4));
     for (int base = 0; base < count; base += D) {
 #pragma unroll
         for (int u = 0; u < D; ++u) {
@@ -249,11 +252,11 @@
         }
     }
 }
-template <int WT, int D, bool SP, int RT>
+template <int WT, int D, bool SP, int RT, bool SWZ = false>
 __device__ __forceinline__ void gemm_split16r(WSplit<WT, D, SP>& ws, const _Float16* Xh, const _Float16* Xl, int ldx,
                                               f32x4 (&am)[RT][WT], f32x4 (&ac)[RT][WT], int step0, int count) {
     const int lane = threadIdx.x & 63;
-    const int off = (lane & 15) * ldx + 8 * (lane >> 4);
+    const int off = (lane & 15) * ldx + 8 * (SWZ ? swz_chunk(lane >> 4, lane & 15) : (lane >> 4));
     for (int base = 0; base < count; base += D) {
 #pragma unroll
         for (int u = 0; u < D; ++u) {
diff --git a/pepflowww_amd/csrc/node_track.hip b/pepflowww_amd/csrc/node_track.hip
--- a/pepflowww_amd/csrc/node_track.hip
+++ b/pepflowww_amd/csrc/node_track.hip
@@ -19,7 +19,8 @@
 
 constexpr int TR = 16;
 constexpr int LDX = 132;
-constexpr int LDP = 136;
+constexpr int LDP = 144;
+constexpr int LDC = 256 + 16;
 constexpr int NTHR = 512;
 #ifndef PF_NT_MINW
 #define PF_NT_MINW 2
@@ -63,10 +64,11 @@
         const float y0[4] = {y[0], y[1], y[2], y[3]}, y1[4] = {y[4], y[5], y[6], y[7]};
         split4(y0, h0, l0);
         split4(y1, h1, l1);
-        *reinterpret_cast<half4*>(out.h + row * LDP + 8 * sub) = h0;
-        *reinterpret_cast<half4*>(out.h + row * LDP + 8 * sub + 4) = h1;
-        *reinterpret_cast<half4*>(out.l + row * LDP + 8 * sub) = l0;
-        *reinterpret_cast<half4*>(out.l + row * LDP + 8 * sub + 4) = l1;
+        const int pc = row * LDP + 8 * swz_chunk(sub, row);
+        *reinterpret_cast<half4*>(out.h + pc) = h0;
+        *reinterpret_cast<half4*>(out.h + pc + 4) = h1;
+        *reinterpret_cast<half4*>(out.l + pc) = l0;
+        *reinterpret_cast<half4*>(out.l + pc + 4) = l1;
         if (gout && m < M) {
             *reinterpret_cast<float4*>(gout + (size_t)m * 128 + 8 * sub) = make_float4(y[0], y[1], y[2], y[3]);
             *reinterpret_cast<float4*>(gout + (size_t)m * 128 + 8 * sub + 4) = make_float4(y[4], y[5], y[6], y[7]);
@@ -82,14 +84,14 @@
 __device__ __forceinline__ void put_planes(Planes p, int r, int n, const float (&v)[4]) {
     half4 hi, lo;
     split4(v, hi, lo);
-    *reinterpret_cast<half4*>(p.h + r * LDP + n) = hi;
-    *reinterpret_cast<half4*>(p.l + r * LDP + n) = lo;
+    *reinterpret_cast<half4*>(p.h + r * LDP + swz_at(n, r)) = hi;
+    *reinterpret_cast<half4*>(p.l + r * LDP + swz_at(n, r)) = lo;
 }
 
 template <bool SP, bool DUMP = false, bool PM = false>
 __global__ __launch_bounds__(NTHR, PF_NT_MINW) void node_head_kernel(pf_node_head_args a) {
     extern __shared__ __attribute__((aligned(16))) unsigned char smem_raw[];
-    constexpr int CK = 256, LDC = CK + 8;
+    constexpr int CK = 256;
     _Float16* Ch = reinterpret_cast<_Float16*>(smem_raw);
     float* X = reinterpret_cast<float*>(smem_raw + 2 * 2 * TR * LDC * sizeof(_Float16));
     Planes Xa = {reinterpret_cast<_Float16*>(X + TR * LDX), reinterpret_cast<_Float16*>(X + TR * LDX) + TR * LDP};
@@ -132,8 +134,8 @@
             const float v[4] = {sv.x, sv.y, sv.z, sv.w};
             half4 hi, lo;
             split4(v, hi, lo);
-            *reinterpret_cast<half4*>(bh + srow * LDC + hlf * 128 + 4 * sc4) = hi;
-            *reinterpret_cast<half4*>(bl + srow * LDC + hlf * 128 + 4 * sc4) = lo;
+            *reinterpret_cast<half4*>(bh + srow * LDC + swz_at(hlf * 128 + 4 * sc4, srow)) = hi;
+            *reinterpret_cast<half4*>(bl + srow * LDC + swz_at(hlf * 128 + 4 * sc4, srow)) = lo;
         }
     };
     if constexpr (PM) {
@@ -150,7 +152,7 @@
 #pragma unroll
     for (int c = C0; c < NCH; ++c) {
         const _Float16* bh = Ch + (c & 1) * 2 * TR * LDC;
-        gemm_split16(ws, bh, bh + TR * LDC, LDC, am, ac, (c - C0) * 8, 8);
+        gemm_split16<1, 8, SP, true>(ws, bh, bh + TR * LDC, LDC, am, ac, (c - C0) * 8, 8);
         if (c + 1 < NCH) commit(c + 1);
         __syncthreads();
     }
@@ -176,7 +178,7 @@
     __syncthreads();
     f32x4 qm[3], qc[3];
     acc_zero1<3>(qm, qc);
-    gemm_split16(wq, Xa.h, Xa.l, LDP, qm, qc, 0, 4);
+    gemm_split16<3, 4, SP, true>(wq, Xa.h, Xa.l, LDP, qm, qc, 0, 4);
     if (mr < M) {
 #pragma unroll
         for (int wt = 0; wt < 3; ++wt) {
@@ -192,7 +194,7 @@
 template <bool SP, bool PM = false>
 __global__ __launch_bounds__(NTHR, PF_NT_MINW) void node_head32_kernel(pf_node_head_args a) {
     extern __shared__ __attribute__((aligned(16))) unsigned char smem_raw[];
-    constexpr int CK = 256, LDC = CK + 8;
+    constexpr int CK = 256;
     _Float16* Ch = reinterpret_cast<_Float16*>(smem_raw);
     float* X = reinterpret_cast<float*>(smem_raw + 2 * 2 * TR2 * LDC * sizeof(_Float16));
     Planes Xa = {reinterpret_cast<_Float16*>(X + TR2 * LDX), reinterpret_cast<_Float16*>(X + TR2 * LDX) + TR2 * LDP};
@@ -246,8 +248,8 @@
             const float v[4] = {sv.x, sv.y, sv.z, sv.w};
             half4 hi, lo;
             split4(v, hi, lo);
-            *reinterpret_cast<half4*>(bh + row * LDC + 4 * c4) = hi;
-            *reinterpret_cast<half4*>(bl + row * LDC + 4 * c4) = lo;
+            *reinterpret_cast<half4*>(bh + row * LDC + swz_at(4 * c4, row)) = hi;
+            *reinterpret_cast<half4*>(bl + row * LDC + swz_at(4 * c4, row)) = lo;
         }
     };
     fetch(0, st[0]);
@@ -282,7 +284,7 @@
     for (int c = C0; c < NCH; ++c) {
         if (!PM && c + 2 < NCH) fetch(c + 2, st[c & 1]);
         const _Float16* bh = Ch + (c & 1) * 2 * TR2 * LDC;
-        gemm_split16r<1, 8, SP, 2>(ws, bh, bh + TR2 * LDC, LDC, am, ac, (c - C0) * 8, 8);
+        gemm_split16r<1, 8, SP, 2, true>(ws, bh, bh + TR2 * LDC, LDC, am, ac, (c - C0) * 8, 8);
         if (c + 1 < NCH) commit(c + 1, st[(c + 1) & 1]);
         __syncthreads();
     }
@@ -310,7 +312,7 @@
     f32x4 qm[2][3], qc[2][3];
 #pragma unroll
     for (int rt = 0; rt < 2; ++rt) acc_zero1<3>(qm[rt], qc[rt]);
-    gemm_split16r<3, 4, SP, 2>(wq, Xa.h, Xa.l, LDP, qm, qc, 0, 4);
+    gemm_split16r<3, 4, SP, 2, true>(wq, Xa.h, Xa.l, LDP, qm, qc, 0, 4);
 #pragma unroll
     for (int rt = 0; rt < 2; ++rt) {
         const int mr = m0 + rt * 16 + r;
@@ -325,6 +327,8 @@
         }
     }
 }
+
+__device__ __forceinline__ int s_xor(int ti, int h) { return (4 * (ti & 3)) ^ (16 * ((ti >> 2) & 1)) ^ (16 * (h >> 1)); }
 
 template <bool LAST, bool SP, int RT, bool DUMP = false>
 __global__ __launch_bounds__(NTHR, PF_NT_MINW) void node_tfmr_kernel(pf_node_tfmr_args a, int LP, int LDS_S) {
@@ -410,21 +414,25 @@
     WSplit<1, 4, SP> ws;
     ws.init(a.w_o_f16, 128, 128, wave * 16);
     ws.prefetch();
-    LnParams ln1, ln2, ln3;
-    ln_load(ln1, a.n1_g, a.n1_b);
-    ln_load(ln2, a.n2_g, a.n2_b);
-    if (LAST) ln_load(ln3, a.nt_g, a.nt_b);
-    const float4 bias_o = *reinterpret_cast<const float4*>(a.b_o + n), bias_1 = *reinterpret_cast<const float4*>(a.b_1 + n),
-                 bias_2 = *reinterpret_cast<const float4*>(a.b_2 + n);
+    const float4 bias_o = *reinterpret_cast<const float4*>(a.b_o + n);
     float4 bias_post = z4, bias_t1 = z4, bias_t2 = z4, bias_t3 = z4, bias_bb = z4, bias_init = z4;
     float4 bias_in[3] = {z4, z4, z4}, bias_pre[4] = {z4, z4, z4, z4};
+    LnParams ln1, ln2, ln3;
+    float4 bias_1 = z4, bias_2 = z4;
     float4 rres_ld[RT], rsipa_ld[RT];
-#pragma unroll
-    for (int rt = 0; rt < RT; ++rt) {
-        const int mrc = mr[rt] < M ? mr[rt] : M - 1;
-        rres_ld[rt] = *reinterpret_cast<const float4*>(a.resid + (size_t)mrc * 128 + n);
-        rsipa_ld[rt] = LAST ? *reinterpret_cast<const float4*>(a.s_ipa + (size_t)mrc * 128 + n) : z4;
-    }
+    auto load_chain_consts = [&]() {
+        ln_load(ln1, a.n1_g, a.n1_b);
+        ln_load(ln2, a.n2_g, a.n2_b);
+        if (LAST) ln_load(ln3, a.nt_g, a.nt_b);
+        bias_1 = *reinterpret_cast<const float4*>(a.b_1 + n);
+        bias_2 = *reinterpret_cast<const float4*>(a.b_2 + n);
+#pragma unroll
+        for (int rt = 0; rt < RT; ++rt) {
+            const int mrc = mr[rt] < M ? mr[rt] : M - 1;
+            rres_ld[rt] = *reinterpret_cast<const float4*>(a.resid + (size_t)mrc * 128 + n);
+            rsipa_ld[rt] = LAST ? *reinterpret_cast<const float4*>(a.s_ipa + (size_t)mrc * 128 + n) : z4;
+        }
+    };
     float lnmask_ld = 1.f;
     const int lnrow = m0 + ((tid & (16 * TR - 1)) >> 4);
     auto load_tail_consts = [&]() {
@@ -440,9 +448,7 @@
         }
         lnmask_ld = a.mask[lnrow < M ? lnrow : M - 1];
     };
-    if (LAST) {
-        if (RT == 1) load_tail_consts();
-    } else {
+    if (!LAST) {
 #pragma unroll
         for (int wt = 0; wt < 3; ++wt) bias_in[wt] = *reinterpret_cast<const float4*>(a.b_in_next + wave * 48 + wt * 16 + 4 * g);
     }
@@ -462,7 +468,7 @@
                         acc = mfma16(q0[rt].x, k0[t].x, acc); acc = mfma16(q0[rt].y, k0[t].y, acc); acc = mfma16(q0[rt].z, k0[t].z, acc); acc = mfma16(q0[rt].w, k0[t].w, acc);
                         acc = mfma16(q1[rt].x, k1[t].x, acc); acc = mfma16(q1[rt].y, k1[t].y, acc); acc = mfma16(q1[rt].z, k1[t].z, acc); acc = mfma16(q1[rt].w, k1[t].w, acc);
 #pragma unroll
-                        for (int e = 0; e < 4; ++e) S[((16 * rt + 4 * g + e) * 4 + h) * LDS_S + j] = keep ? acc[e] * scale : -3.0e38f;
+                        for (int e = 0; e < 4; ++e) S[((16 * rt + 4 * g + e) * 4 + h) * LDS_S + (j ^ s_xor(4 * g + e, h))] = keep ? acc[e] * scale : -3.0e38f;
                     }
                 }
             }
@@ -476,18 +482,24 @@
             score_block(j0, kn0, kn1, knm);
         }
     }
+    asm volatile("" ::: "memory");
+    load_chain_consts();
+    if (LAST && RT == 1) load_tail_consts();
     __syncthreads();
     PROF(2);
 #pragma unroll
     for (int ps = 0; ps < RT; ++ps) {
         const int sub = lane & 7;
-        float* sp = S + ((ps * 8 + wave) * 8 + (lane >> 3)) * LDS_S;
+        const int srow = (ps * 8 + wave) * 8 + (lane >> 3);
+        const int sx = s_xor(srow >> 2, srow & 3);
+        float* sp = S + srow * LDS_S;
+        const int c0 = (4 * sub) ^ sx;
         if (LP <= 256) {
             float4 v[8];
 #pragma unroll
             for (int u = 0; u < 8; ++u) {
                 const int j = 4 * sub + 32 * u;
-                v[u] = j < LP ? *reinterpret_cast<const float4*>(sp + j) : make_float4(-3.0e38f, -3.0e38f, -3.0e38f, -3.0e38f);
+                v[u] = j < LP ? *reinterpret_cast<const float4*>(sp + c0 + 32 * u) : make_float4(-3.0e38f, -3.0e38f, -3.0e38f, -3.0e38f);
             }
             float m = -3.0e38f;
 #pragma unroll
@@ -505,17 +517,17 @@
 #pragma unroll
             for (int u = 0; u < 8; ++u) {
                 const int j = 4 * sub + 32 * u;
-                if (j < LP) *reinterpret_cast<float4*>(sp + j) = make_float4(v[u].x * inv, v[u].y * inv, v[u].z * inv, v[u].w * inv);
+                if (j < LP) *reinterpret_cast<float4*>(sp + c0 + 32 * u) = make_float4(v[u].x * inv, v[u].y * inv, v[u].z * inv, v[u].w * inv);
             }
         } else {
             float m = -3.0e38f;
-            for (int j = sub; j < LP; j += 8) m = fmaxf(m, sp[j]);
+            for (int j = sub; j < LP; j += 8) m = fmaxf(m, sp[j ^ sx]);
             m = fmaxf(m, lane_xor1(m)); m = fmaxf(m, lane_xor2(m)); m = fmaxf(m, lane_xor4(m));
             float sum = 0.f;
-            for (int j = sub; j < LP; j += 8) { const float e = (sp[j] > -1.0e38f) ? exp_softmax(sp[j] - m) : 0.f; sp[j] = e; sum += e; }
+            for (int j = sub; j < LP; j += 8) { const float e = (sp[j ^ sx] > -1.0e38f) ? exp_softmax(sp[j ^ sx] - m) : 0.f; sp[j ^ sx] = e; sum += e; }
             sum += lane_xor1(sum); sum += lane_xor2(sum); sum += lane_xor4(sum);
             const float inv = 1.f / sum;
-            for (int j = sub; j < LP; j += 8) sp[j] *= inv;
+            for (int j = sub; j < LP; j += 8) sp[j ^ sx] *= inv;
         }
     }
     __syncthreads();
@@ -524,14 +536,15 @@
         f32x4 acc[RT];
 #pragma unroll
         for (int rt = 0; rt < RT; ++rt) acc[rt] = (f32x4){0.f, 0.f, 0.f, 0.f};
-        const float* prow = S + (r * 4 + h) * LDS_S + 4 * g;
+        const float* prow = S + (r * 4 + h) * LDS_S;
+        const int px = (4 * g) ^ s_xor(r, h);
         auto pv_block = [&](int k0, const float (&vb)[4][4]) {
 #pragma unroll
             for (int s4 = 0; s4 < 4; ++s4) {
                 if (k0 + 16 * s4 < LP) {
 #pragma unroll
                     for (int rt = 0; rt < RT; ++rt) {
-                        const float4 pa = *reinterpret_cast<const float4*>(prow + rt * 64 * LDS_S + k0 + 16 * s4);
+                        const float4 pa = *reinterpret_cast<const float4*>(prow + rt * 64 * LDS_S + ((k0 + 16 * s4) ^ px));
                         acc[rt] = mfma16(pa.x, vb[s4][0], acc[rt]); acc[rt] = mfma16(pa.y, vb[s4][1], acc[rt]);
                         acc[rt] = mfma16(pa.z, vb[s4][2], acc[rt]); acc[rt] = mfma16(pa.w, vb[s4][3], acc[rt]);
                     }
@@ -551,8 +564,8 @@
 #pragma unroll
             for (int e = 0; e < 4; ++e) {
                 const _Float16 hi = (_Float16)acc[rt][e];
-                Xa.h[(16 * rt + 4 * g + e) * LDP + col] = hi;
-                Xa.l[(16 * rt + 4 * g + e) * LDP + col] = (_Float16)((acc[rt][e] - (float)hi) * PF_LO_SCALE);
+                Xa.h[(16 * rt + 4 * g + e) * LDP + swz_at(col, 4 * g + e)] = hi;
+                Xa.l[(16 * rt + 4 * g + e) * LDP + swz_at(col, 4 * g + e)] = (_Float16)((acc[rt][e] - (float)hi) * PF_LO_SCALE);
                 if constexpr (DUMP) { if (m0 + 16 * rt + 4 * g + e < M) a.dump[0][(size_t)(m0 + 16 * rt + 4 * g + e) * 128 + col] = acc[rt][e]; }
             }
     }
@@ -574,7 +587,7 @@
         for (int e = 0; e < 4; ++e) v[e] = fmaxf(v[e], 0.f);
     };
     zero();
-    gemm_split16r<1, 4, SP, RT>(ws, Xa.h, Xa.l, LDP, am, ac, 0, 4);
+    gemm_split16r<1, 4, SP, RT, true>(ws, Xa.h, Xa.l, LDP, am, ac, 0, 4);
     ws.init(a.w_1_f16, 128, 128, wave * 16);
     ws.prefetch();
 #pragma unroll
@@ -590,7 +603,7 @@
     __syncthreads();
     PROF(5);
     zero();
-    gemm_split16r<1, 4, SP, RT>(ws, Xb.h, Xb.l, LDP, am, ac, 0, 4);
+    gemm_split16r<1, 4, SP, RT, true>(ws, Xb.h, Xb.l, LDP, am, ac, 0, 4);
     ws.init(a.w_2_f16, 128, 128, wave * 16);
     ws.prefetch();
 #pragma unroll
@@ -604,7 +617,7 @@
     __syncthreads();
     PROF(6);
     zero();
-    gemm_split16r<1, 4, SP, RT>(ws, Xa.h, Xa.l, LDP, am, ac, 0, 4);
+    gemm_split16r<1, 4, SP, RT, true>(ws, Xa.h, Xa.l, LDP, am, ac, 0, 4);
     auto lin2_to_t0 = [&]() {
 #pragma unroll
         for (int rt = 0; rt < RT; ++rt) {
@@ -627,7 +640,7 @@
         f32x4 qm[RT][3], qc[RT][3];
 #pragma unroll
         for (int rt = 0; rt < RT; ++rt) acc_zero1<3>(qm[rt], qc[rt]);
-        gemm_split16r<3, 4, SP, RT>(wq, Xb.h, Xb.l, LDP, qm, qc, 0, 4);
+        gemm_split16r<3, 4, SP, RT, true>(wq, Xb.h, Xb.l, LDP, qm, qc, 0, 4);
 #pragma unroll
         for (int rt = 0; rt < RT; ++rt) {
             if (mr[rt] < M) {
@@ -661,7 +674,7 @@
         __syncthreads();
         PROF(7);
         zero();
-        gemm_split16r<1, 4, SP, RT>(ws, Xb.h, Xb.l, LDP, am, ac, 0, 4);
+        gemm_split16r<1, 4, SP, RT, true>(ws, Xb.h, Xb.l, LDP, am, ac, 0, 4);
         ws.init(a.w_t1_f16, 128, 128, wave * 16);
         ws.prefetch();
 #pragma unroll
@@ -677,7 +690,7 @@
         __syncthreads();
         PROF(8);
         zero();
-        gemm_split16r<1, 4, SP, RT>(ws, Xa.h, Xa.l, LDP, am, ac, 0, 4);
+        gemm_split16r<1, 4, SP, RT, true>(ws, Xa.h, Xa.l, LDP, am, ac, 0, 4);
         ws.init(a.w_t2_f16, 128, 128, wave * 16);
         ws.prefetch();
 #pragma unroll
@@ -690,7 +703,7 @@
         }
         __syncthreads();
         zero();
-        gemm_split16r<1, 4, SP, RT>(ws, Xb.h, Xb.l, LDP, am, ac, 0, 4);
+        gemm_split16r<1, 4, SP, RT, true>(ws, Xb.h, Xb.l, LDP, am, ac, 0, 4);
         ws.init(a.w_t3_f16, 128, 128, wave * 16);
         ws.prefetch();
 #pragma unroll
@@ -703,7 +716,7 @@
         }
         __syncthreads();
         zero();
-        gemm_split16r<1, 4, SP, RT>(ws, Xa.h, Xa.l, LDP, am, ac, 0, 4);
+        gemm_split16r<1, 4, SP, RT, true>(ws, Xa.h, Xa.l, LDP, am, ac, 0, 4);
         const bool do_bb = wave == 0, do_init = a.has_et && wave >= 4;
         if (do_bb) { ws.init(a.w_bb_f16, 16, 128, 0); ws.prefetch(); }
         else if (do_init) { ws.init(a.w_init_f16, 64, 128, (wave - 4) * 16); ws.prefetch(); }
@@ -723,7 +736,7 @@
         PROF(9);
         if (do_bb || do_init) {
             zero();
-            gemm_split16r<1, 4, SP, RT>(ws, Xb.h, Xb.l, LDP, am, ac, 0, 4);
+            gemm_split16r<1, 4, SP, RT, true>(ws, Xb.h, Xb.l, LDP, am, ac, 0, 4);
 #pragma unroll
             for (int rt = 0; rt < RT; ++rt) {
                 float v[4];
@@ -755,7 +768,7 @@
 #pragma unroll
             for (int rt = 0; rt < RT; ++rt) acc_zero1<4>(pm[rt], pc[rt]);
             PROF(12);
-            gemm_split16r<4, 2, SP, RT>(wp, Xa.h, Xa.l, LDP, pm, pc, 0, 2);
+            gemm_split16r<4, 2, SP, RT, true>(wp, Xa.h, Xa.l, LDP, pm, pc, 0, 2);
             PROF(13);
 #pragma unroll
             for (int rt = 0; rt < RT; ++rt) {
@@ -771,60 +784,72 @@
             }
         } else if (a.logits_out) {
             __syncthreads();
+            const int net = wave >> 2, wn = wave & 3;
             Planes Xc = {reinterpret_cast<_Float16*>(T0), reinterpret_cast<_Float16*>(T0) + TR * LDP};
-#pragma unroll
-            for (int net = 0; net < 2; ++net) {
-                const int nout = net ? 5 : 20, ntile = net ? 1 : 2;
-                ws.init(a.h_w[net][0], 128, 128, wave * 16);
+            Planes Xd = {reinterpret_cast<_Float16*>(S), reinterpret_cast<_Float16*>(S) + TR * LDP};
+            const Planes h1 = {net ? Xc.h : Xa.h, net ? Xc.l : Xa.l}, h2 = {net ? Xd.h : Xb.h, net ? Xd.l : Xb.l};
+            const int nout = net ? 5 : 20, ntile = net ? 1 : 2;
+            WSplit<2, 4, SP> wh;
+            wh.init(net ? a.h_w[1][0] : a.h_w[0][0], 128, 128, wn * 32);
+            wh.prefetch();
+            float4 hb0[2], hb1[2];
+#pragma unroll
+            for (int wt = 0; wt < 2; ++wt) {
+                hb0[wt] = *reinterpret_cast<const float4*>((net ? a.h_b[1][0] : a.h_b[0][0]) + wn * 32 + 16 * wt + 4 * g);
+                hb1[wt] = *reinterpret_cast<const float4*>((net ? a.h_b[1][1] : a.h_b[0][1]) + wn * 32 + 16 * wt + 4 * g);
+            }
+            f32x4 hm[RT][2], hc[RT][2];
+            auto head_stage_out = [&](const float4 (&bias)[2], Planes out) {
+#pragma unroll
+                for (int rt = 0; rt < RT; ++rt)
+#pragma unroll
+                    for (int wt = 0; wt < 2; ++wt) {
+                        float v[4] = {join(hm[rt][wt], hc[rt][wt], 0) + bias[wt].x, join(hm[rt][wt], hc[rt][wt], 1) + bias[wt].y,
+                                      join(hm[rt][wt], hc[rt][wt], 2) + bias[wt].z, join(hm[rt][wt], hc[rt][wt], 3) + bias[wt].w};
+                        relu4(v);
+                        put_planes(out, 16 * rt + r, wn * 32 + 16 * wt + 4 * g, v);
+                    }
+            };
+#pragma unroll
+            for (int rt = 0; rt < RT; ++rt) acc_zero1<2>(hm[rt], hc[rt]);
+            gemm_split16r<2, 4, SP, RT, true>(wh, Xb.h, Xb.l, LDP, hm, hc, 0, 4);
+            wh.init(net ? a.h_w[1][1] : a.h_w[0][1], 128, 128, wn * 32);
+            wh.prefetch();
+            head_stage_out(hb0, h1);
+            __syncthreads();
+#pragma unroll
+            for (int rt = 0; rt < RT; ++rt) acc_zero1<2>(hm[rt], hc[rt]);
+            gemm_split16r<2, 4, SP, RT, true>(wh, h1.h, h1.l, LDP, hm, hc, 0, 4);
+            const int nl = wn * 16 + 4 * g;
+            float4 hb2 = z4;
+            if (wn < ntile) {
+                ws.init(net ? a.h_w[1][2] : a.h_w[0][2], 16 * ntile, 128, wn * 16);
                 ws.prefetch();
-                const float4 hb0 = *reinterpret_cast<const float4*>(a.h_b[net][0] + n), hb1 = *reinterpret_cast<const float4*>(a.h_b[net][1] + n);
+                hb2 = *reinterpret_cast<const float4*>((net ? a.h_b[1][2] : a.h_b[0][2]) + nl);
+            }
+            head_stage_out(hb1, h2);
+            __syncthreads();
+            if (wn < ntile) {
                 zero();
-                gemm_split16r<1, 4, SP, RT>(ws, Xb.h, Xb.l, LDP, am, ac, 0, 4);
-                ws.init(a.h_w[net][1], 128, 128, wave * 16);
-                ws.prefetch();
+                gemm_split16r<1, 4, SP, RT, true>(ws, h2.h, h2.l, LDP, am, ac, 0, 4);
 #pragma unroll
                 for (int rt = 0; rt < RT; ++rt) {
-                    float v[4];
-                    joined(rt, hb0, v);
-                    relu4(v);
-                    put_planes(Xa, 16 * rt + r, n, v);
-                }
-                __syncthreads();
-                zero();
-                gemm_split16r<1, 4, SP, RT>(ws, Xa.h, Xa.l, LDP, am, ac, 0, 4);
-                if (wave < ntile) { ws.init(a.h_w[net][2], 16 * ntile, 128, wave * 16); ws.prefetch(); }
-#pragma unroll
-                for (int rt = 0; rt < RT; ++rt) {
-                    float v[4];
-                    joined(rt, hb1, v);
-                    relu4(v);
-                    put_planes(Xc, 16 * rt + r, n, v);
-                }
-                __syncthreads();
-                if (wave < ntile) {
-                    const float4 hb2 = *reinterpret_cast<const float4*>(a.h_b[net][2] + n);
-                    zero();
-                    gemm_split16r<1, 4, SP, RT>(ws, Xc.h, Xc.l, LDP, am, ac, 0, 4);
-#pragma unroll
-                    for (int rt = 0; rt < RT; ++rt) {
-                        if (mr[rt] < M) {
-                            float* op = (net ? a.ang_out : a.logits_out) + (size_t)mr[rt] * nout;
-                            float v[4];
-                            joined(rt, hb2, v);
-#pragma unroll
-                            for (int e = 0; e < 4; ++e)
-                                if (n + e < nout) op[n + e] = v[e];
-                        }
+                    if (mr[rt] < M) {
+                        float* op = (net ? a.ang_out : a.logits_out) + (size_t)mr[rt] * nout;
+                        float v[4];
+                        joined(rt, hb2, v);
+#pragma unroll
+                        for (int e = 0; e < 4; ++e)
+                            if (nl + e < nout) op[nl + e] = v[e];
                     }
                 }
-                __syncthreads();
             }
         }
         PROF(11);
     }
 }
 
-constexpr int LDF = 640 + 8;
+constexpr int LDF = 640 + 16;
 template <bool SP>
 __global__ __launch_bounds__(NTHR) void input_mixer_kernel(pf_input_mixer_args a) {
     extern __shared__ __attribute__((aligned(16))) unsigned char smem_raw[];
@@ -884,8 +909,8 @@
         }
         half4 hi, lo;
         split4(v, hi, lo);
-        *reinterpret_cast<half4*>(Xf.h + row * LDF + 4 * c4) = hi;
-        *reinterpret_cast<half4*>(Xf.l + row * LDF + 4 * c4) = lo;
+        *reinterpret_cast<half4*>(Xf.h + row * LDF + swz_at(4 * c4, row)) = hi;
+        *reinterpret_cast<half4*>(Xf.l + row * LDF + swz_at(4 * c4, row)) = lo;
     }
     if (tid < TR && m0 + tid < M) {
         float R[9], q[4];
@@ -897,7 +922,7 @@
     __syncthreads();
     f32x4 am[1], ac[1];
     acc_zero1<1>(am, ac);
-    gemm_split16(w0, Xf.h, Xf.l, LDF, am, ac, 0, 20);
+    gemm_split16<1, 8, SP, true>(w0, Xf.h, Xf.l, LDF, am, ac, 0, 20);
     WSplit<1, 4, SP> w2;
     w2.init(a.w2_f16, 128, 128, wave * 16);
     w2.prefetch();
@@ -908,7 +933,7 @@
     }
     __syncthreads();
     acc_zero1<1>(am, ac);
-    gemm_split16(w2, Xa.h, Xa.l, LDP, am, ac, 0, 4);
+    gemm_split16<1, 4, SP, true>(w2, Xa.h, Xa.l, LDP, am, ac, 0, 4);
     if (mr < M) {
         float4 y;
         y.x = (join(am[0], ac[0], 0) + b2.x) * rmask; y.y = (join(am[0], ac[0], 1) + b2.y) * rmask;
@@ -935,10 +960,10 @@
     if (!a || !a->feats || !a->s_in || !a->mask || !a->w_out_f16 || !a->b_out || !a->ln_g || !a->ln_b || !a->w_in_f16 ||
         !a->b_in || !a->s_ipa || !a->qkv || a->rows <= 0)
         return PF_E_BADARG;
-    const size_t lds = (size_t)2 * 2 * TR * 264 * sizeof(_Float16) + (size_t)TR * LDX * sizeof(float) +
+    const size_t lds = (size_t)2 * 2 * TR * LDC * sizeof(_Float16) + (size_t)TR * LDX * sizeof(float) +
                        (size_t)2 * TR * LDP * sizeof(_Float16);
     if (a->rows >= pf_cu_count() * TR2 && !a->dump_a0) {
-        const size_t lds2 = (size_t)2 * 2 * TR2 * 264 * sizeof(_Float16) + (size_t)TR2 * LDX * sizeof(float) + (size_t)2 * TR2 * LDP * sizeof(_Float16);
+        const size_t lds2 = (size_t)2 * 2 * TR2 * LDC * sizeof(_Float16) + (size_t)TR2 * LDX * sizeof(float) + (size_t)2 * TR2 * LDP * sizeof(_Float16);
         static PfOncePerDevice attr_set;
         if (attr_set.first()) {
             (void)hipFuncSetAttribute((const void*)node_head32_kernel<true>, hipFuncAttributeMaxDynamicSharedMemorySize, 160 * 1024);
@@ -991,7 +1016,7 @@
                 if (!a->h_w[net][l] || !a->h_b[net][l]) return PF_E_BADARG;
     }
     const int LP = (a->L + 15) / 16 * 16;
-    const int LDS_S = LP + 4;
+    const int LDS_S = (LP + 31) / 32 * 32 + 8;
     const int tiles16 = (a->L + 15) / 16;
     auto lds_of = [&](int rt) {
         const int tr = 16 * rt;
```

New measurement: 2.960 million res*step/s, median of 6. About the same (+1.0%).
